# talmolab/Brax-Rodent-Run

Hardware: AMD Instinct MI355X
Metric: env-steps/sec (whole node), rodent 2048 envs/GPU (higher is better)
Workload: dtype f32

## Files before the change

__graft_entry__.py:

```python
import os
import subprocess
import sys

ROOT = os.path.dirname(os.path.abspath(__file__))
PKG = os.path.join(ROOT, "brax-rodent-run_amd")
for p in (ROOT, PKG):
    if p not in sys.path:
        sys.path.insert(0, p)


def build() -> None:
    csrc = os.path.join(PKG, "csrc")
    so = os.path.join(csrc, "librodent_hip.so")
    srcs = [os.path.join(csrc, f) for f in ("rr_api.hip", "rr_kernel.h", "rr_step_body.inc", "rr_mlp.h", "rr_ppo.h", "rr_tanh_normal.h")] + [os.path.join(ROOT, "include", "rodent_rr.h")]
    if not os.path.exists(so) or any(os.path.getmtime(s) > os.path.getmtime(so) for s in srcs):
        cmd = ["hipcc", "--offload-arch=gfx950", "-O2", "-std=c++17", "-shared", "-fPIC", "-fno-slp-vectorize", "-Xclang", "-target-feature",
               "-Xclang", "-load-store-opt", "-o", so, os.path.join(csrc, "rr_api.hip")]
        r = subprocess.run(cmd, stderr=subprocess.PIPE, text=True)
        sys.stderr.write("".join(l for l in r.stderr.splitlines(True) if "not a recognized feature for this target" not in l))
        if r.returncode:
            raise subprocess.CalledProcessError(r.returncode, cmd)
    subprocess.check_call(["make", "-s", "-C", os.path.join(ROOT, "oracle")])
    import rodent_amd
    from rodent_amd import hip
    import ctypes
    lib = ctypes.CDLL(hip.LIB_PATH)
    for sym in hip.EXPORTS:
        getattr(lib, sym)


def smoke() -> None:
    import numpy as np
    import torch
    from rodent_amd import envs, jax_random
    from tests import parity, util
    from tests.oracle_env import OracleRodent

    track = util.synthetic_track()
    N = 64
    env = envs.get_environment("rodent", track_pos=track, num_envs=N, xml_path="rodent_optimized.xml",
                               iterations=8, ls_iterations=8, device="cuda:0")
    keys = jax_random.split(jax_random.PRNGKey(0), N)
    state = env.reset(keys)
    action = parity.f32r(np.random.default_rng(0).uniform(-1, 1, (N, env.action_size)))
    nstate = env.step(state, torch.tensor(action, dtype=torch.float32, device="cuda:0"))
    torch.cuda.synchronize()
    A = OracleRodent("rodent_optimized", N, "f64", (8, 8), track)
    B = OracleRodent("rodent_optimized", N, "f32", (8, 8), track)
    A.reset(keys); B.reset(keys)
    assert np.array_equal(state.pipeline_state.qpos.cpu().numpy(), A.state()["qpos"].astype(np.float32))
    oa, ob = A.step(action), B.step(action)
    assert np.array_equal(nstate.info["cur_frame"].cpu().numpy(), A.cur_frame)
    assert np.array_equal(nstate.done.cpu().numpy(), A.done)
    got = nstate.obs.cpu().numpy().astype(np.float64)
    rows = []
    for k, sl in parity.obs_segments(A.tables).items():
        sc = np.maximum(np.abs(oa[:, sl]).max(1), 1e-3) if k == "cinert" else 1.0
        rows += parity.quantile_rows("obs_" + k, np.abs(got[:, sl] - oa[:, sl]).max(1) / sc, np.abs(ob[:, sl] - oa[:, sl]).max(1) / sc, qs=(0.5,))
    floors = dict(parity.ENV_FLOORS, obs_qpos=parity.ENV_FLOORS["qpos"], obs_qvel=parity.ENV_FLOORS["qvel"])
    parity.check_quantiles(rows, floors)
    assert torch.isfinite(nstate.obs).all()
    print("smoke ok: %d envs, 1 env step (10 substeps); median |qpos - f64 oracle| = %.2e (scalar float32 oracle: %.2e)"
          % (N, rows[0][2], rows[0][3]))


if __name__ == "__main__":
    build()
    if len(sys.argv) > 1 and sys.argv[1] == "smoke":
        smoke()
```

brax-rodent-run_amd/csrc/rr_api.hip:

```cpp
#include "../../include/rodent_rr.h"
#include "rr_kernel.h"
#include "rr_mlp.h"
#include "rr_ppo.h"

#include <atomic>
#include <climits>
#include <cmath>
#include <cstdio>
#include <cstdlib>
#include <cstring>
#include <map>
#include <memory>
#include <mutex>
#include <string>
#include <type_traits>
#include <vector>

static thread_local std::string g_err;
static int fail(int code, const std::string& msg) { g_err = msg; return code; }
extern "C" const char* rr_last_error(void) { return g_err.c_str(); }

#define HIPCHK(x)                                                                                  \
  do {                                                                                             \
    hipError_t e_ = (x);                                                                           \
    if (e_ != hipSuccess) return fail(RR_EHIP, std::string(#x) + ": " + hipGetErrorString(e_));   \
  } while (0)

typedef void (*kern_t)(const RRDims, const RRTables, const RRIO, const int, const int);
struct Entry { int dtype, ndim, dims[4]; size_t count; const void* data; };

struct rr_model {
  std::vector<unsigned char> raw;
  std::map<std::string, Entry> e;
  rr_dims dims;
  RRDims kd;
  std::vector<std::string> dbg_names;
  std::vector<int32_t> dbg_off, dbg_size;
  std::vector<const char*> dbg_cnames;
  int NBS, NVS, NCS;
  bool stage_ok = true;
  int solver = 1;
  bool pair_ok = false;
  RRDims kd_rep;
  bool dyn = false;
  mutable std::atomic<int> live_batches{0};

  const Entry* find(const char* n) const { auto it = e.find(n); return it == e.end() ? nullptr : &it->second; }
  int iscalar(const char* n) const { const Entry* x = find(n); return x ? ((const int32_t*)x->data)[0] : 0; }
  float fscalar(const char* n, int i = 0) const { const Entry* x = find(n); return x ? ((const float*)x->data)[i] : 0.f; }
};

enum Form { F_STEP, F_UNROLL, F_ACTOR, F_EVAL, N_FORMS };
enum Variant { V_PROD, V_DEBUG, V_PROFILE, V_RAND, V_PAIR, V_POSE, N_VARIANTS };
struct Instance { kern_t kern; const char* why = nullptr; bool fixed = false; };

static Instance select(const rr_model* m, Form form, Variant v) {
  const bool s111 = m->NBS == 1 && m->NVS == 1 && m->NCS == 1, s221 = m->NBS == 2 && m->NVS == 2 && m->NCS == 1, s332 = m->NBS == 3 && m->NVS == 3 && m->NCS == 2;
  const bool newton = m->solver == 2, eval = form == F_EVAL, unroll = form != F_STEP, actor = form == F_ACTOR;
  const char *no_diag = "no diagnostic kernel instance for this model", *no_slots = "no kernel instance for this model's slot counts";
  auto no = [](const char* why) { return Instance{nullptr, why}; };
  if (v == V_PAIR && (unroll || newton || !RRDimsRodentNew::matches(m->kd_rep))) return no("no two-wave pair instance for this model / launch form");
  if (v == V_PAIR) return {rr_step_kernel<2, 2, 1, false, false, RRDimsRodentNew, false, false, false, true>, nullptr, true};
  if (unroll && (v == V_DEBUG || v == V_PROFILE)) return no("rr_env_unroll: no diagnostic outputs in a multi-step rollout");
  if (eval) {
    if (newton) return no("rr_env_unroll_eval: the Newton solver has no multi-step instance");
    if (m->pair_ok) return no("rr_env_unroll_eval: two-tree models served by the two-wave pair instance have no multi-step instance");
    if (!s221) return no("rr_env_unroll_eval: only the (2,2,1) slot counts have an evaluation instance");
    if (v == V_RAND) return no("rr_env_unroll_eval: no evaluation instance reads per-env parameters (this batch carries some)");
    if (v == V_POSE) return no("rr_env_unroll_eval: no evaluation instance rewards the pose (this env io carries track_pose); evaluate step by step");
  } else if (v == V_POSE) {
    if (m->dyn) return no("pose tracking: models with candidate-pair contacts (DYN instances) have no pose instance");
    if (m->pair_ok) return no("pose tracking: two-tree models served by the two-wave pair instance have no pose instance");
    if (newton) return no("pose tracking: the Newton solver's instances have no pose instance");
    if (!s221) return no("pose tracking: only the (2,2,1) slot counts have pose instances");
  } else if (v == V_RAND) {
    if (m->dyn) return no("models with candidate-pair contacts (DYN instances) have none");
    if (m->pair_ok) return no("two-tree models served by the two-wave pair instance have none");
    if (newton) return no("the Newton solver's instances have none");
    if (!s221) return no("only the (2,2,1) slot counts have instances with per-env parameters");
  } else if (unroll && (newton || !s221))
    return no("rr_env_unroll: no multi-step kernel instance for this model / solver");
  if (m->dyn) {
    if (v != V_PROD) return no(no_diag);
    if (newton || !s221) return no(no_slots);
    if (eval) return Instance{rr_eval_kernel<RRDims, true>};
    return Instance{actor ? rr_step_kernel<2, 2, 1, false, false, RRDims, false, true, true, false, true>
                    : (unroll ? rr_step_kernel<2, 2, 1, false, false, RRDims, false, true, false, false, true> : rr_step_kernel<2, 2, 1, false, false, RRDims, false, false, false, false, true>)};
  }
  if (v == V_PROFILE && (newton || !s221)) return no(no_diag);
  if (v == V_PROFILE) return RRDimsRodent::matches(m->kd) ? Instance{rr_step_kernel<2, 2, 1, true, false, RRDimsRodent>, nullptr, true} : Instance{rr_step_kernel<2, 2, 1, true, false, RRDims>};
  if (newton)
    return Instance{v == V_DEBUG ? rr_step_kernel<2, 2, 1, false, true, RRDims, true> : rr_step_kernel<2, 2, 1, false, false, RRDims, true>};
  if (v == V_DEBUG)
    return s111 ? Instance{rr_step_kernel<1, 1, 1, false, true, RRDims>} : (s221 ? Instance{rr_step_kernel<2, 2, 1, false, true, RRDims>} : (s332 ? Instance{rr_step_kernel<3, 3, 2, false, true, RRDims>} : no(no_diag)));
  if (!s221) return s111 ? Instance{rr_step_kernel<1, 1, 1, false, false, RRDims>} : (s332 ? Instance{rr_step_kernel<3, 3, 2, false, false, RRDims>} : no(no_slots));
  auto family = [&](auto* t) -> kern_t {
    typedef typename std::remove_pointer<decltype(t)>::type DT;
    if (eval) return rr_eval_kernel<DT>;
    if (v == V_RAND) return actor ? rr_rand_kernel<DT, true, true> : (unroll ? rr_rand_kernel<DT, true> : rr_rand_kernel<DT>);
    if (v == V_POSE) return actor ? rr_pose_kernel<DT, true, true> : (unroll ? rr_pose_kernel<DT, true> : rr_pose_kernel<DT>);
    return actor ? rr_step_kernel<2, 2, 1, false, false, DT, false, true, true> : (unroll ? rr_step_kernel<2, 2, 1, false, false, DT, false, true> : rr_step_kernel<2, 2, 1, false, false, DT>);
  };
  if (RRDimsRodent::matches(m->kd)) return {family((RRDimsRodent*)nullptr), nullptr, true};
  if (RRDimsRodentNew::matches(m->kd)) return {family((RRDimsRodentNew*)nullptr), nullptr, true};
  return Instance{family((RRDims*)nullptr)};
}

static void set_layout(RRDims& k, const RRLayout& L) {
  k.o_qpos = L.o_qpos; k.o_qvel = L.o_qvel; k.o_act = L.o_act; k.o_ctrl = L.o_ctrl; k.o_xpos = L.o_xpos; k.o_xquat = L.o_xquat;
  k.o_cinert = L.o_cinert; k.o_cdof = L.o_cdof; k.o_cvel = L.o_cvel; k.o_qLD = L.o_qLD; k.o_vec = L.o_vec; k.o_x = L.o_x;
  k.o_arm = L.o_arm; k.o_warm = L.o_warm; k.o_qact = L.o_qact; k.o_jlist = L.o_jlist; k.lds_floats = L.lds_floats;
  k.o_H = L.o_H; k.o_Mp = L.o_Mp; k.o_anc = L.o_anc;
}
static bool stage_fits(int nbody, int nv, int con_slots, int nalias) {
  const int pose = std::max(7 * nbody + 4, 6 * nv);
  return 2 * (nalias + 4) <= pose && 2 * (nbody + 8) <= pose && 6 * con_slots <= pose && 4 * con_slots + nv <= std::min(std::min(10 * nbody, 6 * nbody), pose);
}
static bool solve_jobs_fit(const rr_model* m, const char* prefix, int njs, const RRDims& k) {
  return (int)m->find((std::string(prefix) + "k_coljob").c_str())->count == 9 * njs && (int)m->find((std::string(prefix) + "k_rowjob").c_str())->count == 5 * njs &&
         k.lmax <= 16 && k.lmax >= 1 && k.cmax <= 8 && k.rmax <= 8 && k.cmax >= 1;
}

static void layout(rr_model* m) {
  RRDims& k = m->kd;
  const rr_dims& d = m->dims;
  const int con_slots = m->dyn ? m->NCS * RR_LANES : d.ncon;
  const RRLayout L = rr_layout(d.nq, d.nv, d.nu, d.nbody, d.nM, con_slots, m->solver == 2);
  set_layout(k, L);
  k.solver = m->solver;
  k.nfac = m->iscalar(m->solver == 2 ? "k_factor3p_rows" : "k_factor3_rows");
  k.nalias = m->solver == 2 ? 0 : m->iscalar("k_nalias");
  m->dbg_names.clear(); m->dbg_off.clear(); m->dbg_size.clear(); m->dbg_cnames.clear();
  m->stage_ok = stage_fits(d.nbody, d.nv, con_slots, k.nalias);
  if (m->dyn && d.nu > std::max(7 * d.nbody + 4, 6 * d.nv)) m->stage_ok = false;
  int g = 0;
  auto dbg = [&](const char* name, int n) { int r = g; m->dbg_names.push_back(name); m->dbg_off.push_back(g); m->dbg_size.push_back(n); g += n; return r; };
  k.g_xpos = dbg("xpos", 3 * d.nbody); k.g_xquat = dbg("xquat", 4 * d.nbody); k.g_xmat = dbg("xmat", 9 * d.nbody);
  k.g_com = dbg("subtree_com", 6); k.g_cinert = dbg("cinert", 10 * d.nbody); k.g_crb = dbg("crb", 10 * d.nbody);
  k.g_cdof = dbg("cdof", 6 * d.nv); k.g_cvel = dbg("cvel", 6 * d.nbody); k.g_cfrc = dbg("cfrc", 6 * d.nbody);
  k.g_qM = dbg("qM", d.nM); k.g_qLD = dbg("qLD", d.nM); k.g_dinv = dbg("qLDiagInv", d.nv);
  k.g_bias = dbg("qfrc_bias", d.nv); k.g_passive = dbg("qfrc_passive", d.nv); k.g_actuator = dbg("qfrc_actuator", d.nv);
  k.g_smooth = dbg("qfrc_smooth", d.nv); k.g_qacc_smooth = dbg("qacc_smooth", d.nv);
  k.g_con_dist = dbg("con_dist", d.ncon); k.g_con_pos = dbg("con_pos", 3 * d.ncon); k.g_con_frame = dbg("con_frame", 9 * d.ncon);
  k.g_con_D = dbg("con_D", d.ncon); k.g_con_aref = dbg("con_aref", 4 * d.ncon); k.g_lim = dbg("limit_pos_D_aref", 3 * d.nv);
  k.g_qacc = dbg("qacc", d.nv); k.g_qfrc_constraint = dbg("qfrc_constraint", d.nv); k.g_misc = dbg("niter_cost", 2);
  k.g_ls_iters = dbg("ls_iters", 2);
  k.g_solver_end = dbg("solver_end", 2);
  k.g_kaok = dbg("kernarg_ok", 1);
  k.dbg_floats = g;
  for (auto& s : m->dbg_names) m->dbg_cnames.push_back(s.c_str());
  m->dims.lds_bytes = L.lds_floats * (int)sizeof(float);
  m->dims.dbg_floats = g;
  m->dims.solver = m->solver;
  m->dims.fixed_instance = select(m, F_STEP, V_PROD).fixed ? 1 : 0;
}

static void setup_replica(rr_model* m) {
  m->pair_ok = false;
  const char* sw = getenv("RR_PAIR_WAVES");
  if (sw && sw[0] == '0') return;
  static const char* need[] = {"h_dims", "h_k_slots", "h_k_body_i", "h_k_body_f", "h_k_jnt_i", "h_k_jnt_f", "h_k_dof_i", "h_k_dof_f", "h_k_act_f", "h_k_M_ij_k",
                               "h_k_body_anc", "h_k_nround", "h_k_factor3", "h_k_factor3_rows", "h_k_linv", "h_k_linv_rows", "h_k_coljob", "h_k_rowjob", "h_k_jobown",
                               "h_k_solve_lmax", "h_k_solve_cmax", "h_k_solve_rmax", "h_k_nalias", "h_k_con_i", "h_k_con_f", "h_k_con_chain_rows", "h_k_root_mass"};
  for (const char* n : need) if (!m->find(n)) return;
  const int32_t* hd = (const int32_t*)m->find("h_dims")->data;
  const int32_t* sl = (const int32_t*)m->find("h_k_slots")->data;
  if (m->find("h_dims")->count < 8 || sl[0] != 2 || sl[1] != 2 || sl[2] != 1) return;
  if (2 * hd[0] != m->dims.nq || 2 * hd[1] != m->dims.nv || 2 * hd[2] != m->dims.nu || 2 * hd[6] != m->dims.ncon || m->dims.na != m->dims.nu) return;
  RRDims k = m->kd;
  k.nq = hd[0]; k.nv = hd[1]; k.nu = hd[2]; k.nbody = hd[3]; k.njnt = hd[4]; k.nM = hd[5]; k.ncon = hd[6]; k.dmax = hd[7];
  k.nroot = (int)m->find("h_k_root_mass")->count;
  k.nround = m->iscalar("h_k_nround"); k.ninv = m->iscalar("h_k_linv_rows"); k.nfac = m->iscalar("h_k_factor3_rows"); k.nalias = m->iscalar("h_k_nalias");
  k.lmax = m->iscalar("h_k_solve_lmax"); k.cmax = m->iscalar("h_k_solve_cmax"); k.rmax = m->iscalar("h_k_solve_rmax");
  k.obs_dim = k.nq + k.nv + 16 * (k.nbody - 1) + k.nv + 3;
  const RRLayout L = rr_layout(k.nq, k.nv, k.nu, k.nbody, k.nM, k.ncon, false);
  set_layout(k, L);
  k.solver = 1;
  k.nv_scale = m->dims.nv;
  k.lds_bytes_rep = L.lds_floats * 4;
  k.fac_stride = (int)m->find("h_k_factor3")->count; k.inv_stride = (int)m->find("h_k_linv")->count;
  if (!solve_jobs_fit(m, "h_", 2 * RR_LANES, k)) return;
  if (k.nM > RR_LANES * 18 || k.nroot != 1) return;
  if (!stage_fits(k.nbody, k.nv, k.ncon, k.nalias) || 2 * k.lds_bytes_rep + 128 > 64 * 1024) return;
  m->kd_rep = k;
  m->pair_ok = select(m, F_STEP, V_PAIR).kern != nullptr;
}

extern "C" int rr_model_load(const char* path, rr_model** out) {
  if (!path || !out) return fail(RR_EINVAL, "rr_model_load: null argument");
  FILE* f = fopen(path, "rb");
  if (!f) return fail(RR_EIO, std::string("rr_model_load: cannot open ") + path);
  fseek(f, 0, SEEK_END);
  long n = ftell(f);
  fseek(f, 0, SEEK_SET);
  rr_model* m = new rr_model();
  m->raw.resize(n);
  size_t got = fread(m->raw.data(), 1, n, f);
  fclose(f);
  if ((long)got != n || n < 8 || memcmp(m->raw.data(), "RRM1", 4)) { delete m; return fail(RR_EIO, "rr_model_load: not an RRM1 blob"); }
  const unsigned char* raw = m->raw.data();
  uint32_t ne = *(const uint32_t*)(raw + 4);
  if (8 + (size_t)ne * 72 > (size_t)n) { delete m; return fail(RR_EIO, "rr_model_load: truncated header"); }
  const unsigned char* p = raw + 8;
  for (uint32_t i = 0; i < ne; ++i, p += 72) {
    Entry e;
    char name[33] = {0};
    memcpy(name, p, 32);
    e.dtype = *(const uint32_t*)(p + 32);
    e.ndim = *(const uint32_t*)(p + 36);
    for (int k = 0; k < 4; ++k) e.dims[k] = *(const uint32_t*)(p + 40 + 4 * k);
    uint64_t off = *(const uint64_t*)(p + 56), nb = *(const uint64_t*)(p + 64);
    if (off + nb > (uint64_t)n) { delete m; return fail(RR_EIO, "rr_model_load: entry out of range"); }
    e.count = nb / 4;
    e.data = raw + off;
    m->e[name] = e;
  }
  static const char* need[] = {"nq", "nv", "nu", "nbody", "njnt", "ngeom", "nM", "ncon", "nlimit", "nefc", "obs_dim", "k_slots",
                               "k_body_i", "k_body_f", "k_jnt_i", "k_jnt_f", "k_dof_i", "k_dof_f", "k_act_f", "k_M_ij_k", "k_body_anc",
                               "k_nround", "k_factor3", "k_factor3_rows", "k_factor3p", "k_factor3p_rows", "k_nalias", "k_linv", "k_linv_rows", "k_coljob", "k_rowjob",
                               "k_jobown", "k_solve_lmax", "k_solve_cmax", "k_solve_rmax", "k_con_i", "k_con_f", "k_con_chain_packed", "k_con_chain_rows", "k_root_mass",
                               "k_act_i", "k_act_m_i", "k_act_m_f",
                               "dof_depth", "body_depth", "opt_timestep", "opt_gravity", "stat_meaninertia"};
  for (const char* nme : need)
    if (!m->find(nme)) { std::string s = std::string("rr_model_load: blob lacks '") + nme + "'"; delete m; return fail(RR_EIO, s); }
  rr_dims& d = m->dims;
  memset(&d, 0, sizeof(d));
  d.nq = m->iscalar("nq"); d.nv = m->iscalar("nv"); d.nu = m->iscalar("nu"); d.na = m->iscalar("na"); d.nbody = m->iscalar("nbody");
  d.njnt = m->iscalar("njnt"); d.ngeom = m->iscalar("ngeom"); d.nM = m->iscalar("nM"); d.ncon = m->iscalar("ncon");
  d.nlimit = m->iscalar("nlimit"); d.nefc = m->iscalar("nefc"); d.obs_dim = m->iscalar("obs_dim");
  d.iterations = m->iscalar("opt_iterations"); d.ls_iterations = m->iscalar("opt_ls_iterations");
  d.timestep = m->fscalar("opt_timestep");
  const int32_t* sl = (const int32_t*)m->find("k_slots")->data;
  m->NBS = sl[0]; m->NVS = sl[1]; m->NCS = sl[2];
  m->dyn = m->iscalar("k_dyn") != 0;
  if (m->dyn && (m->find("k_con_i")->dims[1] != 8 || m->find("k_con_f")->dims[1] != 32 || (int)m->find("k_con_chain_rows")->count != 10 * (d.ncon + 1) || d.nv >= 128 || d.nu > RR_LANES)) {
    delete m; return fail(RR_EIO, "rr_model_load: candidate-pair tables do not match the DYN kernel instance (stale blob)"); }
  RRDims& k = m->kd;
  memset(&k, 0, sizeof(k));
  k.nq = d.nq; k.nv = d.nv; k.nu = d.nu; k.nbody = d.nbody; k.njnt = d.njnt; k.nM = d.nM; k.ncon = d.ncon;
  int dmax = 0;
  { const Entry* dd = m->find("dof_depth"); for (size_t i = 0; i < dd->count; ++i) dmax = std::max(dmax, ((const int32_t*)dd->data)[i]); }
  k.dmax = dmax;
  k.nroot = (int)m->find("k_root_mass")->count;
  k.nround = m->iscalar("k_nround");
  k.ninv = m->iscalar("k_linv_rows");
  if (d.nM > RR_LANES * (m->NVS == 1 ? 10 : (m->NVS == 2 ? 18 : 35))) { delete m; return fail(RR_EUNSUPPORTED, "rr_model_load: more mass-matrix entries than the kernel's register table"); }
  k.lmax = m->iscalar("k_solve_lmax"); k.cmax = m->iscalar("k_solve_cmax"); k.rmax = m->iscalar("k_solve_rmax");
  if (!solve_jobs_fit(m, "", (m->NVS >= 3 ? m->NVS + 1 : m->NVS) * RR_LANES, k)) {
    delete m; return fail(RR_EIO, "rr_model_load: solve job tables do not match the kernel instance (stale blob)"); }
  k.obs_dim = d.obs_dim; k.iterations = d.iterations; k.ls_iterations = d.ls_iterations;
  k.dt = d.timestep; k.gx = m->fscalar("opt_gravity", 0); k.gy = m->fscalar("opt_gravity", 1); k.gz = m->fscalar("opt_gravity", 2);
  k.tolerance = m->fscalar("opt_tolerance"); k.ls_tolerance = m->fscalar("opt_ls_tolerance");
  k.meaninertia = m->fscalar("stat_meaninertia");
  if (k.nroot > 2) { delete m; return fail(RR_EUNSUPPORTED, "rr_model_load: more than 2 kinematic trees"); }
  if (m->find("k_dof_i")->dims[1] != RR_DOFI) { delete m; return fail(RR_EIO, "rr_model_load: k_dof_i width mismatch (stale blob)"); }
  if (m->find("k_body_i")->dims[1] != RR_BODYI) { delete m; return fail(RR_EIO, "rr_model_load: k_body_i width mismatch (stale blob)"); }
  if (d.nv > 256 || (!m->dyn && d.ncon > 256)) { delete m; return fail(RR_EUNSUPPORTED, "rr_model_load: nv/ncon above the 8-bit table index"); }
  if (m->find("k_con_chain_packed")->dims[1] != m->NCS * RR_LANES) { delete m; return fail(RR_EIO, "rr_model_load: lane-table width mismatch"); }
  k.nv_scale = d.nv > 1 ? d.nv : 1;
  layout(m);
  setup_replica(m);
  *out = m;
  return RR_OK;
}

extern "C" int rr_model_dims(const rr_model* m, rr_dims* out) {
  if (!m || !out) return fail(RR_EINVAL, "rr_model_dims: null argument");
  *out = m->dims;
  return RR_OK;
}
extern "C" int rr_model_set_solver(rr_model* m, int32_t it, int32_t ls) {
  if (!m || it < 0 || ls < 0) return fail(RR_EINVAL, "rr_model_set_solver: bad argument");
  m->dims.iterations = m->kd.iterations = it;
  m->dims.ls_iterations = m->kd.ls_iterations = ls;
  return RR_OK;
}
extern "C" int rr_model_set_solver_type(rr_model* m, int32_t solver) {
  if (!m || (solver != 1 && solver != 2)) return fail(RR_EINVAL, "rr_model_set_solver_type: solver must be 1 (cg) or 2 (newton)");
  if (solver != m->solver && m->live_batches.load() > 0)
    return fail(RR_EINVAL, "rr_model_set_solver_type: batches of this model exist (they hold the LDS layout of the current solver); set the solver before rr_batch_create");
  if (solver == 2 && (!(m->NBS == 2 && m->NVS == 2 && m->NCS == 1) || m->dyn))
    return fail(RR_EUNSUPPORTED, "rr_model_set_solver_type: the Newton instance exists for the single-rodent models only");
  if (solver == 2 && 4 * ((m->dims.nv + 3) & ~3) > std::max(7 * m->dims.nbody + 4, 6 * m->dims.nv))
    return fail(RR_EUNSUPPORTED, "rr_model_set_solver_type: the four Hessian rows do not fit the pose cells");
  m->solver = solver;
  layout(m);
  return RR_OK;
}
extern "C" void rr_model_destroy(rr_model* m) { delete m; }
extern "C" int rr_model_table(const rr_model* m, const char* name, const void** host_ptr, size_t* count, int32_t* dtype) {
  if (!m || !name || !host_ptr) return fail(RR_EINVAL, "rr_model_table: null argument");
  const Entry* e = m->find(name);
  if (!e) return fail(RR_EINVAL, std::string("rr_model_table: the model has no table '") + name + "'");
  *host_ptr = e->data;
  if (count) *count = e->count;
  if (dtype) *dtype = e->dtype;
  return RR_OK;
}
extern "C" int rr_kernarg_layout(int32_t* io_offset, int32_t* io_size, int32_t* total_size) {
  if (io_offset) *io_offset = (int32_t)offsetof(RRKArgs, io);
  if (io_size) *io_size = (int32_t)sizeof(RRIO);
  if (total_size) *total_size = (int32_t)sizeof(RRKArgs);
  return RR_OK;
}

struct rr_batch {
  const rr_model* m;
  int N, device;
  hipStream_t stream;
  RRDims kd;
  RRTables T;
  RRTables T_rep;
  std::vector<void*> dev_allocs;
  bool timing = false;
  std::vector<hipEvent_t> ev0, ev1;
  int npending = 0, ring_head = 0;
  double total_ms = 0;
  int64_t launches = 0;
  unsigned long long* prof = nullptr;
  const int32_t* env_map = nullptr;
  uint32_t* cost = nullptr;
  bool counted = false;
  unsigned* dyn_overflow = nullptr;
  unsigned* bad_states = nullptr;
  unsigned* progress = nullptr;
  float *env_dof_f = nullptr, *env_act_f = nullptr, *env_con_f = nullptr;
  int dbg_flags = 0;
  float* eval_actions = nullptr;
  rr_pose_io pose = {};
  bool has_env_params() const { return env_dof_f || env_act_f || env_con_f; }
};

template <typename Ptr>
static int dev_alloc(rr_batch* b, size_t bytes, Ptr* dst, const void* host = nullptr, size_t host_bytes = 0) {
  void* p = nullptr;
  HIPCHK(hipMalloc(&p, bytes));
  b->dev_allocs.push_back(p);
  if (host_bytes) HIPCHK(hipMemcpy(p, host, host_bytes, hipMemcpyHostToDevice));
  *dst = (Ptr)p;
  return RR_OK;
}
template <typename Ptr>
static int upload(rr_batch* b, const char* name, Ptr* dst) {
  const Entry* e = b->m->find(name);
  return dev_alloc(b, std::max<size_t>(e->count, 1) * 4, dst, e->data, e->count * 4);
}

static int upload_levels(rr_batch* b, const char* name, rr_gi* dst, uint32_t base, uint32_t alias_base, uint32_t nM, int copies = 1, uint32_t rep_bytes = 0) {
  const Entry* e = b->m->find(name);
  std::vector<uint32_t> t((size_t)copies * e->count);
  for (int c = 0; c < copies; ++c) {
    const uint32_t* src = (const uint32_t*)e->data;
    uint32_t* tc = t.data() + (size_t)c * e->count;
    const uint32_t cb = base + (uint32_t)c * rep_bytes, ab = alias_base + (uint32_t)c * rep_bytes;
    for (size_t i = 0; i + 3 < e->count; i += 4) {
      uint32_t f[6] = {src[i] & 0xFFFFu, src[i] >> 16, src[i + 1] & 0xFFFFu, src[i + 1] >> 16, src[i + 2] & 0xFFFFu, src[i + 2] >> 16};
      for (uint32_t& v : f) {
        v = v < nM + 4u ? v * 8u + cb : (v - (nM + 4u)) * 8u + ab;
        if (v > 0xFFFFu) return fail(RR_EUNSUPPORTED, "level schedule does not fit the 16-bit LDS address fields");
      }
      const uint32_t q = src[i + 3];
      if (q > 255u) return fail(RR_EIO, "level schedule: pivot offset out of range (stale blob)");
      tc[i] = f[0] | (f[1] << 16); tc[i + 1] = f[2] | (f[3] << 16); tc[i + 2] = f[4] | (f[5] << 16);
      tc[i + 3] = q * 8u;
    }
  }
  return dev_alloc(b, t.size() * 4, dst, t.data(), t.size() * 4);
}

static int lds_bytes(const rr_model* m, Variant v) { return v == V_PAIR ? 2 * m->kd_rep.lds_bytes_rep + 128 : m->dims.lds_bytes; }

extern "C" int rr_batch_create(const rr_model* m, int32_t num_envs, int32_t device, void* stream, rr_batch** out) {
  if (!m || !out || num_envs <= 0) return fail(RR_EINVAL, "rr_batch_create: bad argument");
  const Instance prod = select(m, F_STEP, V_PROD);
  if (!prod.kern) return fail(RR_EUNSUPPORTED, std::string("rr_batch_create: ") + prod.why);
  HIPCHK(hipSetDevice(device));
  std::unique_ptr<rr_batch, void (*)(rr_batch*)> guard(new rr_batch(), rr_batch_destroy);
  rr_batch* b = guard.get();
  b->m = m; b->N = num_envs; b->device = device; b->stream = (hipStream_t)stream; b->kd = m->kd;
  int rc = 0;
#define UP(T, prefix, field) if ((rc = upload(b, prefix "k_" #field, &T.field))) return rc;
#define UP_REPLICA_TABLES(T, prefix)                                                                                                \
  UP(T, prefix, body_i) UP(T, prefix, jnt_i) UP(T, prefix, dof_i) UP(T, prefix, M_ij_k) UP(T, prefix, body_anc)                     \
  UP(T, prefix, con_chain_rows) UP(T, prefix, coljob) UP(T, prefix, rowjob) UP(T, prefix, jobown) UP(T, prefix, con_i)              \
  UP(T, prefix, body_f) UP(T, prefix, jnt_f) UP(T, prefix, dof_f) UP(T, prefix, act_f) UP(T, prefix, con_f) UP(T, prefix, root_mass)
  UP_REPLICA_TABLES(b->T, "")
  UP(b->T, "", act_i) UP(b->T, "", act_m_i) UP(b->T, "", act_m_f)
  const uint32_t qb = (uint32_t)m->kd.o_qLD * 4u, ab = (uint32_t)m->kd.o_xpos * 4u, nM = (uint32_t)m->dims.nM;
  if ((rc = upload_levels(b, m->solver == 2 ? "k_factor3p" : "k_factor3", &b->T.factor3, qb, ab, nM)) || (rc = upload_levels(b, "k_linv", &b->T.linv, qb, ab, nM))) return rc;
  memset(&b->T_rep, 0, sizeof(b->T_rep));
  if (m->pair_ok) {
    UP_REPLICA_TABLES(b->T_rep, "h_")
    const uint32_t base = (uint32_t)m->kd_rep.o_qLD * 4u, rb = (uint32_t)m->kd_rep.lds_bytes_rep;
    const uint32_t abase = (uint32_t)m->kd_rep.o_xpos * 4u, hnM = (uint32_t)m->kd_rep.nM;
    if ((rc = upload_levels(b, "h_k_factor3", &b->T_rep.factor3, base, abase, hnM, 2, rb)) || (rc = upload_levels(b, "h_k_linv", &b->T_rep.linv, base, abase, hnM, 2, rb))) return rc;
    b->T_rep.anc4 = b->T_rep.M_ij_k;
  }
#undef UP_REPLICA_TABLES
#undef UP
  {
    const Entry *an = m->find("dof_anc"), *ad = m->find("dof_ancadr"), *ma = m->find("dof_Madr");
    std::vector<unsigned char> bytes(((size_t)m->dims.nM + 3) / 4 * 4 + 4, 0);
    if (an && ad && ma) {
      const int32_t *anc = (const int32_t*)an->data, *adr = (const int32_t*)ad->data, *madr = (const int32_t*)ma->data;
      for (int i = 0; i < m->dims.nv; ++i) {
        const int n = adr[i + 1] - adr[i];
        for (int p = 0; p < n; ++p) bytes[madr[i] + p] = (unsigned char)anc[adr[i] + n - 1 - p];
      }
    } else if (m->solver == 2) return fail(RR_EIO, "rr_batch_create: blob lacks the ancestor tables the Newton solver needs");
    if ((rc = dev_alloc(b, bytes.size(), &b->T.anc4, bytes.data(), bytes.size()))) return rc;
  }
  if (!m->stage_ok) return fail(RR_EUNSUPPORTED, "rr_batch_create: 4*ncon + nv exceeds the line-search staging cells (6*nbody)");
  if (m->dims.lds_bytes > 64 * 1024) return fail(RR_EUNSUPPORTED, "rr_batch_create: per-env working set exceeds the 64 KiB of LDS one workgroup may address");
  for (int f = 0; f < N_FORMS; ++f)
    for (int v = 0; v < N_VARIANTS; ++v) {
      const kern_t kk = select(m, (Form)f, (Variant)v).kern;
      if (!kk) continue;
      HIPCHK(hipFuncSetAttribute((const void*)kk, hipFuncAttributeMaxDynamicSharedMemorySize, lds_bytes(m, (Variant)v)));
      hipFuncAttributes fa;
      HIPCHK(hipFuncGetAttributes(&fa, (const void*)kk));
      if (fa.sharedSizeBytes != 0) return fail(RR_EUNSUPPORTED, "rr_batch_create: a step-kernel instance has static LDS (the level schedules need the dynamic segment at address 0)");
    }
  if (m->dyn && (rc = dev_alloc(b, 64, &b->dyn_overflow))) return rc;
  if (m->dyn) HIPCHK(hipMemset(b->dyn_overflow, 0, 64));
  if ((rc = dev_alloc(b, 64, &b->bad_states))) return rc;
  HIPCHK(hipMemset(b->bad_states, 0, 64));
  const char* pace = getenv("RR_PACE");
  if (!(pace && pace[0] == '0') && (rc = dev_alloc(b, 64, &b->progress))) return rc;
  m->live_batches.fetch_add(1);
  b->counted = true;
  *out = guard.release();
  return RR_OK;
}

extern "C" void rr_batch_destroy(rr_batch* b) {
  if (!b) return;
  if (b->counted) b->m->live_batches.fetch_sub(1);
  for (void* p : b->dev_allocs) (void)hipFree(p);
  for (float* p : {b->env_dof_f, b->env_act_f, b->env_con_f, b->eval_actions}) if (p) (void)hipFree(p);
  for (hipEvent_t e : b->ev0) (void)hipEventDestroy(e);
  for (hipEvent_t e : b->ev1) (void)hipEventDestroy(e);
  delete b;
}

#define RR_TIMING_RING 256
static int collect_timing(rr_batch* b, bool all = true) {
  bool first = true;
  while (b->npending > 0) {
    const int i = b->ring_head;
    if (all || (first && hipEventQuery(b->ev1[i]) != hipSuccess)) HIPCHK(hipEventSynchronize(b->ev1[i]));
    else if (hipEventQuery(b->ev1[i]) != hipSuccess) break;
    first = false;
    float ms = 0;
    HIPCHK(hipEventElapsedTime(&ms, b->ev0[i], b->ev1[i]));
    b->total_ms += ms;
    b->launches += 1;
    b->ring_head = (i + 1) % RR_TIMING_RING;
    b->npending -= 1;
  }
  (void)hipGetLastError();
  return RR_OK;
}

struct Launch {
  int mode = 1;
  const rr_state *st = nullptr, *st_in = nullptr;
  const float* ctrl = nullptr;
  int n_frames = 1;
  const rr_env_io* env = nullptr;
  const int32_t* cur_frame_in = nullptr;
  const rr_outputs* out = nullptr;
  const rr_unroll_io* un = nullptr;
  int unroll_T = 0;
  const rr_actor_io* ac = nullptr;
  const rr_eval_io* ev = nullptr;
};
static int check_wrap(const char* who, const rr_unroll_io* w, const char* note = "") {
  if (!w || !w->first.qpos || !w->first.qvel || !w->first.act || !w->first.qacc_warmstart || !w->first_obs || !w->prev_done || !w->steps_in ||
// ... 732 lines not shown
  }
  b->prof = (unsigned long long*)dev_cycles;
  return RR_OK;
}

extern "C" int rr_batch_env_params_supported(const rr_batch* b) {
  if (!b) return fail(RR_EINVAL, "rr_batch_env_params_supported: null batch");
  return select(b->m, F_STEP, V_RAND).kern ? 1 : 0;
}
extern "C" int rr_batch_pose_supported(const rr_batch* b) {
  if (!b) return fail(RR_EINVAL, "rr_batch_pose_supported: null batch");
  const Instance in = select(b->m, F_STEP, V_POSE);
  const char* why = in.kern ? nullptr : in.why;
  if (!why && b->has_env_params()) why = "pose tracking: no pose instance reads per-env parameters (this batch carries some)";
  if (!why && b->prof) why = "pose tracking: no profile build with track_pose";
  if (why) (void)fail(RR_EUNSUPPORTED, std::string("rr_batch_pose_supported: ") + why);
  return why ? 0 : 1;
}
extern "C" int rr_batch_set_pose(rr_batch* b, const rr_pose_io* p) {
  if (!b) return fail(RR_EINVAL, "rr_batch_set_pose: null batch");
  if (!p || (!p->track_pose && !p->pose_metrics)) { b->pose = rr_pose_io{}; return RR_OK; }
  if (!p->track_pose || !p->pose_metrics) return fail(RR_EINVAL, "rr_batch_set_pose: track_pose and pose_metrics go together");
  for (float x : {p->quat_reward_weight, p->quat_reward_scale, p->joint_reward_weight, p->joint_reward_scale})
    if (!(x >= 0.0f) || !std::isfinite(x)) return fail(RR_EINVAL, "rr_batch_set_pose: pose reward weights and scales must be finite and >= 0");
  if (rr_batch_pose_supported(b) != 1) return RR_EUNSUPPORTED;
  b->pose = *p;
  return RR_OK;
}
extern "C" int rr_batch_set_env_params(rr_batch* b, const rr_env_params* p) {
  if (!b) return fail(RR_EINVAL, "rr_batch_set_env_params: null batch");
  const rr_dims& d = b->m->dims;
  const bool any = p && (p->dof_f || p->act_f || p->con_f);
  if (any) {
    const Instance in = select(b->m, F_STEP, V_RAND);
    if (!in.kern) return fail(RR_EUNSUPPORTED, std::string("rr_batch_set_env_params: no kernel instance with per-env parameters: ") + in.why);
    if (b->prof) return fail(RR_EUNSUPPORTED, "rr_batch_set_env_params: no profile build on a batch with per-env parameters (rr_batch_set_profile is on)");
    if (b->pose.track_pose) return fail(RR_EUNSUPPORTED, "rr_batch_set_env_params: pose tracking: no pose instance reads per-env parameters (rr_batch_set_pose is on)");
    if (p->num_envs != b->N) return fail(RR_EINVAL, "rr_batch_set_env_params: num_envs differs from the batch's");
    if ((p->dof_f && p->dof_rows != d.nv) || (p->act_f && p->act_rows != d.nu) || (p->con_f && p->con_rows != d.ncon))
      return fail(RR_EINVAL, "rr_batch_set_env_params: row counts must be the model's nv (dof_f), nu (act_f), ncon (con_f)");
  }
  HIPCHK(hipSetDevice(b->device));
  HIPCHK(hipStreamSynchronize(b->stream));
  float** own[3] = {&b->env_dof_f, &b->env_act_f, &b->env_con_f};
  for (float** o : own) { if (*o) { HIPCHK(hipFree(*o)); *o = nullptr; } }
  if (!any) return RR_OK;
  const float* src[3] = {p->dof_f, p->act_f, p->con_f};
  const size_t bytes[3] = {(size_t)b->N * d.nv * 16 * 4, (size_t)b->N * d.nu * 8 * 4, (size_t)b->N * d.ncon * 26 * 4};
  for (int i = 0; i < 3; ++i) {
    if (!src[i] || !bytes[i]) continue;
    void* q = nullptr;
    HIPCHK(hipMalloc(&q, bytes[i]));
    *own[i] = (float*)q;
    HIPCHK(hipMemcpyAsync(q, src[i], bytes[i], hipMemcpyDeviceToDevice, b->stream));
  }
  HIPCHK(hipStreamSynchronize(b->stream));
  return RR_OK;
}

extern "C" int rr_batch_set_schedule(rr_batch* b, const int32_t* env_map, uint32_t* cost_cycles) {
  if (!b) return fail(RR_EINVAL, "rr_batch_set_schedule: null batch");
  b->env_map = env_map; b->cost = cost_cycles;
  return RR_OK;
}

extern "C" int rr_batch_set_ls_repeat_exit(rr_batch* b, int32_t enable) {
  if (!b) return fail(RR_EINVAL, "rr_batch_set_ls_repeat_exit: null batch");
  b->dbg_flags = enable ? (b->dbg_flags & ~RR_DBG_LS_RUN_REPEATS) : (b->dbg_flags | RR_DBG_LS_RUN_REPEATS);
  return RR_OK;
}

extern "C" int rr_batch_set_solver_trim(rr_batch* b, int32_t enable) {
  if (!b) return fail(RR_EINVAL, "rr_batch_set_solver_trim: null batch");
  b->dbg_flags = enable ? (b->dbg_flags & ~RR_DBG_SOLVER_UNTRIMMED) : (b->dbg_flags | RR_DBG_SOLVER_UNTRIMMED);
  return RR_OK;
}

extern "C" int rr_batch_set_solver_batch(rr_batch* b, int32_t enable) {
  if (!b) return fail(RR_EINVAL, "rr_batch_set_solver_batch: null batch");
  b->dbg_flags = enable ? (b->dbg_flags & ~RR_DBG_SOLVER_UNBATCHED) : (b->dbg_flags | RR_DBG_SOLVER_UNBATCHED);
  return RR_OK;
}

extern "C" int rr_batch_set_timing(rr_batch* b, int32_t enable) {
  if (!b) return fail(RR_EINVAL, "rr_batch_set_timing: null batch");
  HIPCHK(hipSetDevice(b->device));
  if (enable && b->ev0.empty()) {
    for (int i = 0; i < RR_TIMING_RING; ++i) {
      hipEvent_t a, c;
      HIPCHK(hipEventCreate(&a)); b->ev0.push_back(a);
      HIPCHK(hipEventCreate(&c)); b->ev1.push_back(c);
    }
  }
  b->timing = enable != 0;
  b->total_ms = 0; b->launches = 0; b->npending = 0; b->ring_head = 0;
  return RR_OK;
}
extern "C" int rr_batch_kernel_time(rr_batch* b, double* total_ms, int64_t* launches) {
  if (!b) return fail(RR_EINVAL, "rr_batch_kernel_time: null batch");
  int rc = collect_timing(b);
  if (rc) return rc;
  if (total_ms) *total_ms = b->total_ms;
  if (launches) *launches = b->launches;
  return RR_OK;
}
```

brax-rodent-run_amd/csrc/rr_kernel.h:

```cpp
#pragma once
#include <hip/hip_runtime.h>
#include <stdint.h>
#include "rr_tanh_normal.h"

#define RR_LANES 64
#define RR_DOFI 12
#define RR_BODYI 12
#ifndef RR_WIDE
#define RR_WIDE 1
#endif
#ifndef RR_RING
#define RR_RING 6
#endif

#define RR_NPH 24
#ifndef RR_W1
#define RR_W1 2
#define RR_W2 6
#define RR_W3 12
#endif
#ifndef RR_ENV_PRIO
#define RR_ENV_PRIO 1
#endif
#ifndef RR_FACTOR_PRIO
#define RR_FACTOR_PRIO 1
#endif
#ifndef RR_DPP_BLOCK
#define RR_DPP_BLOCK 1
#endif
#ifndef RR_LS_REPEAT_EXIT
#define RR_LS_REPEAT_EXIT 1
#endif
#ifndef RR_JOBS_RESIDENT
#define RR_JOBS_RESIDENT 1
#endif
#ifndef RR_LS_STAGE_ONCE
#define RR_LS_STAGE_ONCE 1
#endif
#define RR_MINVAL 1e-15f
#define RR_MINIMP 0.0001f
#define RR_MAXIMP 0.9999f

struct RRDims {
  int nq, nv, nu, nbody, njnt, nM, ncon, dmax, nroot;
  int obs_dim, iterations, ls_iterations, nfac, nround, ninv, lmax, cmax, rmax;
  float dt, gx, gy, gz, tolerance, ls_tolerance, meaninertia;
  int o_qpos, o_qvel, o_act, o_ctrl, o_xpos, o_xquat, o_cinert, o_cdof, o_cvel,
      o_qLD, o_vec, o_x, o_arm, o_warm, o_qact, o_jlist, lds_floats;
  int o_H, o_Mp, o_anc, solver;
  int nv_scale, fac_stride, inv_stride, lds_bytes_rep;
  int nalias;
  int g_xpos, g_xquat, g_xmat, g_com, g_cinert, g_crb, g_cdof, g_cvel, g_cfrc, g_qM, g_qLD, g_dinv, g_bias, g_passive,
      g_actuator, g_smooth, g_qacc_smooth, g_con_dist, g_con_pos, g_con_frame, g_con_D, g_con_aref, g_lim, g_qacc,
      g_qfrc_constraint, g_misc, g_ls_iters, g_solver_end, g_kaok, dbg_floats;
};

struct RRLayout {
  int o_qpos, o_qvel, o_act, o_ctrl, o_xpos, o_xquat, o_cinert, o_cdof, o_cvel, o_qLD, o_vec, o_x, o_arm, o_warm, o_qact, o_jlist, lds_floats;
  int o_H, o_Mp, o_anc;
};
constexpr int rr_imax(int a, int b) { return a > b ? a : b; }
constexpr int rr_up4(int n) { return (n + 3) & ~3; }
constexpr RRLayout rr_layout(int nq, int nv, int nu, int nbody, int nM, int ncon, bool newton = false) {
  RRLayout k{};
  int o = 0;
  k.o_qpos = o; o += rr_up4(nq);
  k.o_qvel = o; o += rr_up4(nv + 1);
  k.o_act = o; o += rr_up4(nu);
  k.o_ctrl = o; o += rr_up4(nu);
  k.o_xpos = o; o += rr_up4(rr_imax(7 * nbody + 4, 6 * nv));
  k.o_xquat = k.o_xpos + rr_up4(3 * nbody);
  k.o_cinert = o; o += rr_up4(10 * nbody);
  k.o_cdof = o; o += rr_up4(6 * nv + 6);
  k.o_cvel = o; o += rr_up4(6 * nbody);
  k.o_qLD = o; o += rr_up4(rr_imax(rr_imax(2 * (nM + 20), 12 * nbody), 2 * nv));
  k.o_vec = o; o += rr_up4(nv + 16);
  k.o_x = o; o += rr_up4(nv + 16);
  k.o_arm = o; o += rr_up4(2 * nv);
  k.o_warm = o; o += rr_up4(nv);
  k.o_qact = o; o += rr_up4(nv);
  k.o_jlist = o; o += rr_up4(ncon);
  if (newton) {
    k.o_H = o; o += rr_up4(rr_imax(rr_imax(2 * (nM + 20), 12 * nbody), 2 * nv));
    k.o_Mp = o; o += rr_up4(rr_imax(rr_imax(2 * (nM + 20), 12 * nbody), 2 * nv));
    k.o_anc = o; o += rr_up4((nM + 3) / 4 + 1);
  }
  k.lds_floats = o;
  return k;
}

template <int NBODY_, int NCON_, int OBS_>
struct RRDimsFixed : RRDims {
  static constexpr int nq = 74, nv = 73, nu = 30, nbody = NBODY_, njnt = 68, nM = 1119, ncon = NCON_, dmax = 35, nroot = 1, obs_dim = OBS_, nround = 6, lmax = 12, cmax = 6, rmax = 3;
  static constexpr RRLayout LY = rr_layout(nq, nv, nu, nbody, nM, ncon);
  static constexpr int o_qpos = LY.o_qpos, o_qvel = LY.o_qvel, o_act = LY.o_act, o_ctrl = LY.o_ctrl, o_xpos = LY.o_xpos, o_xquat = LY.o_xquat,
                       o_cinert = LY.o_cinert, o_cdof = LY.o_cdof, o_cvel = LY.o_cvel, o_qLD = LY.o_qLD, o_vec = LY.o_vec,
                       o_x = LY.o_x, o_arm = LY.o_arm, o_warm = LY.o_warm, o_qact = LY.o_qact, o_jlist = LY.o_jlist,
                       lds_floats = LY.lds_floats;
  __host__ __device__ RRDimsFixed(const RRDims& d) : RRDims(d) {}
  static bool matches(const RRDims& d) {
    const RRDims& r = d;
    return r.nq == nq && r.nv == nv && r.nu == nu && r.nbody == nbody && r.njnt == njnt && r.nM == nM && r.ncon == ncon && r.dmax == dmax &&
           r.nroot == nroot && r.obs_dim == obs_dim && r.nround == nround && r.lmax == lmax && r.cmax == cmax && r.rmax == rmax && r.o_qpos == o_qpos && r.o_qvel == o_qvel && r.o_act == o_act &&
           r.o_ctrl == o_ctrl && r.o_xpos == o_xpos && r.o_xquat == o_xquat && r.o_cinert == o_cinert && r.o_cdof == o_cdof &&
           r.o_cvel == o_cvel && r.o_qLD == o_qLD && r.o_vec == o_vec && r.o_x == o_x && r.o_arm == o_arm &&
           r.o_warm == o_warm && r.o_qact == o_qact && r.o_jlist == o_jlist && r.lds_floats == lds_floats;
  }
};
typedef RRDimsFixed<66, 59, 1263> RRDimsRodent;
typedef RRDimsFixed<67, 57, 1279> RRDimsRodentNew;

typedef const int __attribute__((address_space(1)))* rr_gi;
typedef const float __attribute__((address_space(1)))* rr_gf;
struct RRTables {
  rr_gi factor3, linv, coljob, rowjob, jobown, body_i, jnt_i, dof_i, M_ij_k, body_anc, con_chain_rows, con_i, anc4;
  rr_gf body_f, jnt_f, dof_f, act_f, con_f, root_mass;
  rr_gi act_i, act_m_i;
  rr_gf act_m_f;
};
struct RRLoopTables { rr_gi factor3, linv, coljob, rowjob, jobown, con_chain_rows; };
static __device__ __forceinline__ RRTables load_tables();
static __device__ __forceinline__ RRDims load_dims();
static __device__ __forceinline__ RRTables load_env_tables(int env, int nv, int nu, int ncon);
typedef const char __attribute__((address_space(1)))* rr_gc;
template <class E>
struct rr_row {
  rr_gc base; unsigned off; int k0;
  __device__ __forceinline__ E operator[](int k) const { return *(const E __attribute__((address_space(1)))*)(base + (size_t)off + (ptrdiff_t)sizeof(E) * (k0 + k)); }
  __device__ __forceinline__ rr_row operator+(int k) const { return rr_row{base, off, k0 + k}; }
};
__device__ __forceinline__ rr_row<int> row_at(rr_gi t, int stride, int idx) { return rr_row<int>{(rr_gc)t, (unsigned)idx * (4u * (unsigned)stride), 0}; }
__device__ __forceinline__ rr_row<float> row_at(rr_gf t, int stride, int idx) { return rr_row<float>{(rr_gc)t, (unsigned)idx * (4u * (unsigned)stride), 0}; }

#define RR_EVAL_RAW 1
#define RR_EVAL_ACTIONS 2
struct RRIO {
  float *qpos, *qvel, *act, *warm;
  const float *qpos_in, *qvel_in, *act_in, *warm_in;
  const int* cur_frame_in;
  const float* ctrl;
  float *o_cinert, *o_cvel, *o_qfrc_actuator, *o_xpos, *o_xmat, *o_com, *dbg;
  float *o_cdist, *o_cpos, *o_cframe;
  const float* track_pos;
  int track_len;
  int* cur_frame;
  float *obs, *reward, *done, *metrics;
  float healthy_reward, ctrl_cost_weight, z_min, z_max;
  int terminate_when_unhealthy;
  unsigned long long* prof;
  const int* env_map;
  unsigned* cost;
  const float *first_qpos, *first_qvel, *first_act, *first_warm, *first_obs;
  const float *prev_done, *steps_in;
  float *steps_out, *trunc_out;
  float episode_length;
  int unroll_T;
  const float *a_obs_in;
  const float *a_mean, *a_std;
  const float *a_W0, *a_b0;
  const float *a_Wt[4], *a_b[4];
  const float *a_Wth, *a_bh;
  const float *a_noise;
  float *a_actions;
  float *t_obs, *t_raw, *t_logp, *t_reward, *t_discount, *t_trunc;
  float a_min_std;
  int a_nh;
  int a_seg, a_pad;
  unsigned* progress;
  unsigned* dyn_overflow;
  unsigned* bad_states;
  float pace_t1, pace_t2, pace_t3;
  int pace_mode;
  const float* env_dof_f;
  const float* env_act_f;
  const float* env_con_f;
  float* e_metrics;
  float* e_qpos_out;
  int mode;
  float bad_state_max;
  int dbg_flags;
  int num_clips;
  const int* clip;
  const float* track_pose;
  float* pose_metrics;
  float pose_quat_w, pose_quat_k, pose_joint_w, pose_joint_k;
};

#define RR_DBG_LS_RUN_REPEATS 1
#define RR_DBG_SOLVER_UNTRIMMED 2
#define RR_DBG_SOLVER_UNBATCHED 4
struct v3 { float x, y, z; };
__device__ __forceinline__ v3 mk3(float x, float y, float z) { v3 r; r.x = x; r.y = y; r.z = z; return r; }
__device__ __forceinline__ v3 ld3(const float* p) { return mk3(p[0], p[1], p[2]); }
__device__ __forceinline__ v3 ld3(const float __attribute__((address_space(1)))* p) { return mk3(p[0], p[1], p[2]); }
__device__ __forceinline__ v3 ld3(const rr_row<float>& p) { return mk3(p[0], p[1], p[2]); }
__device__ __forceinline__ void st3(float* p, v3 a) { p[0] = a.x; p[1] = a.y; p[2] = a.z; }
__device__ __forceinline__ v3 operator+(v3 a, v3 b) { return mk3(a.x + b.x, a.y + b.y, a.z + b.z); }
__device__ __forceinline__ v3 operator-(v3 a, v3 b) { return mk3(a.x - b.x, a.y - b.y, a.z - b.z); }
__device__ __forceinline__ v3 operator*(v3 a, float s) { return mk3(a.x * s, a.y * s, a.z * s); }
__device__ __forceinline__ float dot(v3 a, v3 b) { return a.x * b.x + a.y * b.y + a.z * b.z; }
__device__ __forceinline__ v3 cross(v3 a, v3 b) { return mk3(a.y * b.z - a.z * b.y, a.z * b.x - a.x * b.z, a.x * b.y - a.y * b.x); }

__device__ __forceinline__ void quat_mul(float* r, const float* a, const float* b) {
  float w = a[0] * b[0] - a[1] * b[1] - a[2] * b[2] - a[3] * b[3];
  float x = a[0] * b[1] + a[1] * b[0] + a[2] * b[3] - a[3] * b[2];
  float y = a[0] * b[2] - a[1] * b[3] + a[2] * b[0] + a[3] * b[1];
  float z = a[0] * b[3] + a[1] * b[2] - a[2] * b[1] + a[3] * b[0];
  r[0] = w; r[1] = x; r[2] = y; r[3] = z;
}
__device__ __forceinline__ void quat_to_mat(float* m, const float* q) {
  float w = q[0], x = q[1], y = q[2], z = q[3];
  m[0] = w * w + x * x - y * y - z * z; m[1] = 2 * (x * y - w * z); m[2] = 2 * (x * z + w * y);
  m[3] = 2 * (x * y + w * z); m[4] = w * w - x * x + y * y - z * z; m[5] = 2 * (y * z - w * x);
  m[6] = 2 * (x * z - w * y); m[7] = 2 * (y * z + w * x); m[8] = w * w - x * x - y * y + z * z;
}
__device__ __forceinline__ v3 mat_vec(const float* m, v3 v) {
  return mk3(m[0] * v.x + m[1] * v.y + m[2] * v.z, m[3] * v.x + m[4] * v.y + m[5] * v.z, m[6] * v.x + m[7] * v.y + m[8] * v.z);
}
__device__ __forceinline__ void quat_normalize(float* q) {
  float n = sqrtf(q[0] * q[0] + q[1] * q[1] + q[2] * q[2] + q[3] * q[3]);
  if (n < RR_MINVAL) { q[0] = 1; q[1] = q[2] = q[3] = 0; return; }
  const float inv = 1.0f / n;
  q[0] *= inv; q[1] *= inv; q[2] *= inv; q[3] *= inv;
}
__device__ __forceinline__ void mul_inert_vec(float* res, const float* i, const float* v) {
  res[0] = i[0] * v[0] + i[3] * v[1] + i[4] * v[2] - i[8] * v[4] + i[7] * v[5];
  res[1] = i[3] * v[0] + i[1] * v[1] + i[5] * v[2] + i[8] * v[3] - i[6] * v[5];
  res[2] = i[4] * v[0] + i[5] * v[1] + i[2] * v[2] - i[7] * v[3] + i[6] * v[4];
  res[3] = i[8] * v[1] - i[7] * v[2] + i[9] * v[3];
  res[4] = i[6] * v[2] - i[8] * v[0] + i[9] * v[4];
  res[5] = i[7] * v[0] - i[6] * v[1] + i[9] * v[5];
}
__device__ __forceinline__ void cross_motion(float* res, const float* vel, const float* v) {
  res[0] = -vel[2] * v[1] + vel[1] * v[2];
  res[1] = vel[2] * v[0] - vel[0] * v[2];
  res[2] = -vel[1] * v[0] + vel[0] * v[1];
  res[3] = -vel[2] * v[4] + vel[1] * v[5] - vel[5] * v[1] + vel[4] * v[2];
  res[4] = vel[2] * v[3] - vel[0] * v[5] + vel[5] * v[0] - vel[3] * v[2];
  res[5] = -vel[1] * v[3] + vel[0] * v[4] - vel[4] * v[0] + vel[3] * v[1];
}
__device__ __forceinline__ void cross_force(float* res, const float* vel, const float* f) {
  res[0] = -vel[2] * f[1] + vel[1] * f[2] - vel[5] * f[4] + vel[4] * f[5];
  res[1] = vel[2] * f[0] - vel[0] * f[2] + vel[5] * f[3] - vel[3] * f[5];
  res[2] = -vel[1] * f[0] + vel[0] * f[1] - vel[4] * f[3] + vel[3] * f[4];
  res[3] = -vel[2] * f[4] + vel[1] * f[5];
  res[4] = vel[2] * f[3] - vel[0] * f[5];
  res[5] = -vel[1] * f[3] + vel[0] * f[4];
}
__device__ __forceinline__ float dot6(const float* a, const float* b) {
  float s = a[0] * b[0];
  s += a[1] * b[1]; s += a[2] * b[2]; s += a[3] * b[3]; s += a[4] * b[4]; s += a[5] * b[5];
  return s;
}
__device__ __forceinline__ float dpp_add(float v, const int ctrl_tag) {
  int x = __float_as_int(v), y;
  switch (ctrl_tag) {
    case 0: y = __builtin_amdgcn_update_dpp(0, x, 0xB1, 0xF, 0xF, true); break;
    case 1: y = __builtin_amdgcn_update_dpp(0, x, 0x4E, 0xF, 0xF, true); break;
    case 2: y = __builtin_amdgcn_update_dpp(0, x, 0x141, 0xF, 0xF, true); break;
    case 3: y = __builtin_amdgcn_update_dpp(0, x, 0x140, 0xF, 0xF, true); break;
    case 4: asm("s_nop 1\n\tv_add_f32_dpp %0, %0, %0 row_bcast:15 row_mask:0xa bank_mask:0xf" : "+v"(v)); return v;
    case 5: asm("s_nop 1\n\tv_add_f32_dpp %0, %0, %0 row_bcast:31 row_mask:0xc bank_mask:0xf" : "+v"(v)); return v;
    default: return v;
  }
  return v + __int_as_float(y);
}
__device__ __forceinline__ float wave_sum(float v) {
  v = dpp_add(v, 0); v = dpp_add(v, 1); v = dpp_add(v, 2); v = dpp_add(v, 3); v = dpp_add(v, 4); v = dpp_add(v, 5);
  return __int_as_float(__builtin_amdgcn_readlane(__float_as_int(v), 63));
}
template <int K>
__device__ __forceinline__ void dpp_bcast_stage(float* v) {
  static_assert(K == 3 || K == 4 || K == 6, "instantiated widths");
// ... 628 lines not shown
  static __device__ __forceinline__ void lds_st2(int byte_adr, rr_f2 v) { *(rr_lf2)(size_t)(unsigned)byte_adr = v; }
  struct RowAdr { int a8, p8, b8, d8[4]; };
  template <bool DIV, bool SHIFT>
  static __device__ __forceinline__ RowAdr row_adr(const rr_v4i& e, int delta) {
    const int sh = SHIFT ? delta : 0;
    RowAdr r;
    r.a8 = (e.x & 0xFFFF) + sh; r.b8 = (int)((unsigned)e.x >> 16) + sh;
    r.p8 = DIV ? r.a8 - e.w + 8 : 0;
    r.d8[0] = (e.y & 0xFFFF) + sh; r.d8[1] = (int)((unsigned)e.y >> 16) + sh; r.d8[2] = (e.z & 0xFFFF) + sh; r.d8[3] = (int)((unsigned)e.z >> 16) + sh;
    return r;
  }
  template <bool DIV, bool SHIFT = false>
  __device__ __forceinline__ void run_levels(rr_gi table, int nrows, int delta = 0) {
    typedef const rr_v4i __attribute__((address_space(1)))* rr_gv4;
    typedef const char __attribute__((address_space(1)))* rr_gc;
    const rr_gc tab = (rr_gc)table;
    const unsigned lane16 = 16u * (unsigned)lane;
    constexpr int ROWB = RR_LANES * 16;
    rr_v4i ring[RR_RING];
#pragma unroll
    for (int u = 0; u < RR_RING; ++u) ring[u] = *(rr_gv4)(tab + u * ROWB + lane16);
    RowAdr cur = row_adr<DIV, SHIFT>(ring[0], delta);
    for (int r0 = 0; r0 < nrows; r0 += RR_RING) {
      const rr_gc nxt_rows = tab + (size_t)(r0 + RR_RING) * ROWB;
#pragma unroll
#if RR_WIDE == 2
      for (int u = 0; u < RR_RING; u += 2) {
        if (u && r0 + u >= nrows) break;
        const RowAdr c0 = cur, c1 = row_adr<DIV, SHIFT>(ring[u + 1], delta);
        const rr_f2 va0 = lds_ld2(c0.a8), va1 = lds_ld2(c1.a8);
        rr_f2 vp0 = {1.0f, 1.0f}, vp1 = {1.0f, 1.0f};
        if (DIV) { vp0 = lds_ld2(c0.p8); vp1 = lds_ld2(c1.p8); }
        rr_f2 vb0[4], vo0[4], vb1[4], vo1[4];
#pragma unroll
        for (int j = 0; j < 4; ++j) vb0[j] = lds_ld2(c0.b8 + 8 * j);
#pragma unroll
        for (int j = 0; j < 4; ++j) vo0[j] = lds_ld2(c0.d8[j]);
#pragma unroll
        for (int j = 0; j < 4; ++j) vb1[j] = lds_ld2(c1.b8 + 8 * j);
#pragma unroll
        for (int j = 0; j < 4; ++j) vo1[j] = lds_ld2(c1.d8[j]);
        ring[u] = *(rr_gv4)(nxt_rows + u * ROWB + lane16);
        ring[u + 1] = *(rr_gv4)(nxt_rows + (u + 1) * ROWB + lane16);
        const RowAdr nxt = row_adr<DIV, SHIFT>(ring[(u + 2) % RR_RING], delta);
        rr_f2 t0 = va0, t1 = va1;
        if (DIV) {
          rr_f2 r0_ = {__builtin_amdgcn_rcpf(vp0.x), __builtin_amdgcn_rcpf(vp0.y)}, r1_ = {__builtin_amdgcn_rcpf(vp1.x), __builtin_amdgcn_rcpf(vp1.y)};
          r0_ = r0_ * (2.0f - vp0 * r0_); r1_ = r1_ * (2.0f - vp1 * r1_);
          t0 *= r0_; t1 *= r1_;
        }
#pragma unroll
        for (int j = 0; j < 4; ++j) lds_st2(c0.d8[j], vo0[j] - vb0[j] * t0);
#pragma unroll
        for (int j = 0; j < 4; ++j) lds_st2(c1.d8[j], vo1[j] - vb1[j] * t1);
        cur = nxt;
      }
      if (true) continue;
#endif
      for (int u = 0; u < RR_RING; ++u) {
        if (u && r0 + u >= nrows) break;
        const rr_f2 va = lds_ld2(cur.a8);
        rr_f2 vp = {1.0f, 1.0f};
        if (DIV) vp = lds_ld2(cur.p8);
        rr_f2 vb[4], vo[4];
#pragma unroll
        for (int j = 0; j < 4; ++j) vb[j] = lds_ld2(cur.b8 + 8 * j);
#pragma unroll
        for (int j = 0; j < 4; ++j) vo[j] = lds_ld2(cur.d8[j]);
        ring[u] = *(rr_gv4)(nxt_rows + u * ROWB + lane16);
        const RowAdr nxt = row_adr<DIV, SHIFT>(ring[(u + 1) % RR_RING], delta);
        rr_f2 t = va;
        if (DIV) {
          rr_f2 r = {__builtin_amdgcn_rcpf(vp.x), __builtin_amdgcn_rcpf(vp.y)};
          r = r * (2.0f - vp * r);
          t *= r;
        }
#pragma unroll
        for (int j = 0; j < 4; ++j) lds_st2(cur.d8[j], vo[j] - vb[j] * t);
        cur = nxt;
      }
    }
  }

  __device__ __forceinline__ void factor() {
    int ment[NME];
    load_ment(ment);
    const RRTables T = tables();
    const DT D = phase_dims();
    if (lane < 8) s_qLD[2 * D.nM + lane] = (lane >> 1) == 1 ? 1.0f : ((lane >> 1) == 3 ? -1.0f : 0.0f);
    for (int c = lane; c < 2 * D.nalias; c += RR_LANES) s_buf[c] = 0.0f;
#pragma unroll
    for (int s = 0; s < NVS; ++s) {
      const int d = lane + RR_LANES * s;
      if (d < D.nv) s_qLD[2 * (opaque(dofc1[s]) & 0xFFFF) + 1] += D.dt * row_at(T.dof_f, 16, d)[1];
    }
    sync();
    run_levels<true>(PAIR ? TL.factor3 + rep * D.fac_stride : TL.factor3, D.nfac);
    sync();
#pragma unroll
    for (int s = 0; s < NVS; ++s) {
      const int d = lane + RR_LANES * s;
      const rr_f2 dd = d < D.nv ? *(const rr_f2*)(s_qLD + 2 * (opaque(dofc1[s]) & 0xFFFF)) : rr_f2{1.0f, 1.0f};
      dinv[s] = d < D.nv ? 1.0f / dd.x : 0.0f;
      dinvB[s] = d < D.nv ? 1.0f / dd.y : 0.0f;
      if (d < D.nv) *(rr_f2*)(s_buf + 2 * d) = rr_f2{dinv[s], dinvB[s]};
    }
    sync();
#pragma unroll
    for (int it = 0; it < NME; ++it) {
      const int ij = ment[it];
      if (ij >= 0) {
        const int i = ij & 255, j = ij >> 8;
        if (i != j) *(rr_f2*)(s_qLD + 2 * (lane + RR_LANES * it)) *= *(const rr_f2*)(s_buf + 2 * i);
      }
    }
    sync();
  }

  __device__ __forceinline__ void invert() {
    const DT D = phase_dims();
    run_levels<false>(PAIR ? TL.linv + rep * D.inv_stride : TL.linv, D.ninv);
  }

  static constexpr int NJS = NVS >= 3 ? NVS + 1 : NVS;
  struct Jobs { int cw[NJS][8], ci0[NJS], rb[NJS][4], ra[NJS], own[NVS]; };
  __device__ __forceinline__ void load_jobs(Jobs& j) { load_jobs(j, TL.coljob, TL.rowjob, TL.jobown); }
  template <class P>
  __device__ __forceinline__ void load_jobs(Jobs& j, P coljob, P rowjob, P jobown) {
    constexpr int WJ = NJS * RR_LANES;
    const int ol = opaque(lane);
    const rr_row<int> cj = row_at(coljob, 1, ol), rj = row_at(rowjob, 1, ol), jo = row_at(jobown, 1, ol);
#pragma unroll
    for (int s = 0; s < NJS; ++s) {
#pragma unroll
      for (int k = 0; k < 8; ++k) j.cw[s][k] = 2 * k < D.lmax ? cj[k * WJ + s * RR_LANES] : 0;
      j.ci0[s] = cj[8 * WJ + s * RR_LANES];
#pragma unroll
      for (int k = 0; k < 4; ++k) j.rb[s][k] = 4 * k < D.lmax ? rj[k * WJ + s * RR_LANES] : 0;
      j.ra[s] = rj[4 * WJ + s * RR_LANES];
    }
#pragma unroll
    for (int s = 0; s < NVS; ++s) j.own[s] = ol + RR_LANES * s < D.nv ? jo[RR_LANES * s] : 0;
  }
  static constexpr bool JOBS_RES = RR_JOBS_RESIDENT != 0 && JRES;
  Jobs jobs_res;
  __device__ __forceinline__ void load_jobs_resident() {
    if constexpr (JOBS_RES) { const RRTables T = load_tables(); load_jobs(jobs_res, T.coljob, T.rowjob, T.jobown); }
  }
  __device__ __forceinline__ void jobs_fresh() {
    constexpr bool ALL = rr_same<DT, RRDims>::value;
#pragma unroll
    for (int s = 0; s < NJS; ++s) {
#pragma unroll
      for (int k = 0; k < 8; ++k) if (ALL || 2 * k < D.lmax) asm volatile("" : "+v"(jobs_res.cw[s][k]));
      asm volatile("" : "+v"(jobs_res.ci0[s]));
#pragma unroll
      for (int k = 0; k < 4; ++k) if (ALL || 4 * k < D.lmax) asm volatile("" : "+v"(jobs_res.rb[s][k]));
      asm volatile("" : "+v"(jobs_res.ra[s]));
    }
#pragma unroll
    for (int s = 0; s < NVS; ++s) asm volatile("" : "+v"(jobs_res.own[s]));
  }
  __device__ __forceinline__ float col_piece(const Jobs& j, int s, const float* mat, const float* vec) const {
    const float* v = vec + j.ci0[s];
    float acc = 0.0f;
#pragma unroll
    for (int t = 0; t < 16; ++t)
      if (t < D.lmax) acc += *(const float*)((const char*)mat + ((j.cw[s][t >> 1] >> (16 * (t & 1))) & 0xFFFF)) * v[t];
    return acc;
  }
  __device__ __forceinline__ float row_piece(const Jobs& j, int s, const float* mat, const float* vec) const {
    const float* m_ = (const float*)((const char*)mat + j.ra[s]);
    float acc = 0.0f;
#pragma unroll
    for (int t = 0; t < 16; ++t)
      if (t < D.lmax) acc += m_[2 * t] * vec[(j.rb[s][t >> 2] >> (8 * (t & 3))) & 255];
    return acc;
  }
  static __device__ __forceinline__ float merge_pieces(const float* part, int t0, int c, int cmax) {
    float sum = 0.0f;
// ... 512 lines not shown
      }
    }
#pragma unroll
    for (int s = 0; s < NVS; ++s) {
      float qcs = qc[s];
      if (lim_act[s] && lim_jar[s] < 0) {
        const float f = -lim_D[s] * lim_jar[s];
        part[0] += lim_D[s] * lim_jar[s] * lim_jar[s];
        qcs += lim_sign[s] * f;
      }
      qfrc_con[s] = qcs;
      part[1] += (Ma[s] - qfrc_smooth[s]) * (qacc[s] - qacc_smooth[s]);
    }
    solver_sum_n<2>(part);
    gauss = 0.5f * part[1];
    prev_cost = cost;
    cost = 0.5f * part[0] + gauss;
  }

  __device__ __forceinline__ void newton_hessian() {
    const int RS = (D.nv + 3) & ~3;
    for (int e = lane; e < D.nM + 20; e += RR_LANES) *(rr_f2*)(s_H + 2 * e) = *(const rr_f2*)(s_Mp + 2 * e);
    float cd[NVS][6];
#pragma unroll
    for (int s = 0; s < NVS; ++s) {
      const int d = lane + RR_LANES * s;
#pragma unroll
      for (int k = 0; k < 6; ++k) cd[s][k] = d < D.nv ? s_cdof[6 * d + k] : 0.0f;
    }
    sync();
#pragma unroll
    for (int s = 0; s < NVS; ++s) {
      if (lim_act[s] && lim_jar[s] < 0) { rr_f2* h = (rr_f2*)(s_H + 2 * (opaque(dofc1[s]) & 0xFFFF)); *h += rr_f2{lim_D[s], lim_D[s]}; }
    }
#pragma unroll
    for (int cs = 0; cs < NCS; ++cs) {
      unsigned long long mask = __ballot(con_act[cs]);
      while (mask) {
        const int l = __builtin_ctzll(mask);
        mask &= mask - 1;
        auto bc = [&](float v) { return __int_as_float(__builtin_amdgcn_readlane(__float_as_int(v), l)); };
        const float mu = bc(con_mu[cs]), Dc = bc(con_D[cs]);
        const v3 off = mk3(bc(con_off[cs][0]), bc(con_off[cs][1]), bc(con_off[cs][2]));
        const v3 fn = mk3(bc(con_fr[cs][0]), bc(con_fr[cs][1]), bc(con_fr[cs][2])), f1 = mk3(bc(con_fr[cs][3]), bc(con_fr[cs][4]), bc(con_fr[cs][5])),
                 f2 = mk3(bc(con_fr[cs][6]), bc(con_fr[cs][7]), bc(con_fr[cs][8]));
        float a[4];
#pragma unroll
        for (int k = 0; k < 4; ++k) a[k] = bc(con_jar[cs][k]) < 0 ? Dc : 0.0f;
        const int ld = __builtin_amdgcn_readlane(con_leaf[cs], l);
        float r[NVS][4];
        bool on[NVS];
#pragma unroll
        for (int s = 0; s < NVS; ++s) {
          const int d = lane + RR_LANES * s;
          on[s] = d < D.nv && d <= ld && ld <= (opaque(dofc1[s]) >> 16);
          const v3 jp = mk3(cd[s][3], cd[s][4], cd[s][5]) + cross(mk3(cd[s][0], cd[s][1], cd[s][2]), off);
          const float jn = dot(fn, jp), j1 = dot(f1, jp), j2 = dot(f2, jp);
          r[s][0] = on[s] ? jn + mu * j1 : 0.0f; r[s][1] = on[s] ? jn - mu * j1 : 0.0f;
          r[s][2] = on[s] ? jn + mu * j2 : 0.0f; r[s][3] = on[s] ? jn - mu * j2 : 0.0f;
          if (d < D.nv) {
#pragma unroll
            for (int k = 0; k < 4; ++k) s_buf[k * RS + d] = r[s][k];
          }
        }
        sync();
#pragma unroll
        for (int s = 0; s < NVS; ++s) {
          if (s > 0 && ld < RR_LANES * s) continue;
          if (on[s]) {
            const int madr = opaque(dofc1[s]) & 0xFFFF, dep = opaque(dofc0[s]) & 255;
            const float w0 = a[0] * r[s][0], w1 = a[1] * r[s][1], w2 = a[2] * r[s][2], w3 = a[3] * r[s][3];
            for (int p = 0; p <= dep; ++p) {
              const int j = s_anc[madr + p];
              const float v = w0 * s_buf[j] + w1 * s_buf[RS + j] + w2 * s_buf[2 * RS + j] + w3 * s_buf[3 * RS + j];
              rr_f2* h = (rr_f2*)(s_H + 2 * (madr + p));
              *h += rr_f2{v, v};
            }
          }
        }
        sync();
      }
    }
  }
  __device__ __forceinline__ void newton_factor() {
    const int delta = (int)((D.o_H - D.o_qLD) * sizeof(float));
    int ment[NME];
    load_ment(ment);
    if (lane < 8) s_H[2 * D.nM + lane] = (lane >> 1) == 1 ? 1.0f : 0.0f;
    sync();
    run_levels<true, true>(TL.factor3, D.nfac, delta);
    sync();
#pragma unroll
    for (int s = 0; s < NVS; ++s) {
      const int d = lane + RR_LANES * s;
      dinvH[s] = d < D.nv ? 1.0f / s_H[2 * (opaque(dofc1[s]) & 0xFFFF)] : 0.0f;
      if (d < D.nv) *(rr_f2*)(s_buf + 2 * d) = rr_f2{dinvH[s], dinvH[s]};
    }
    sync();
#pragma unroll
    for (int it = 0; it < NME; ++it) {
      const int ij = ment[it];
      if (ij >= 0) {
        const int i = ij & 255, j = ij >> 8;
        if (i != j) *(rr_f2*)(s_H + 2 * (lane + RR_LANES * it)) *= *(const rr_f2*)(s_buf + 2 * i);
      }
    }
    sync();
    run_levels<false, true>(TL.linv, D.ninv, delta);
    sync();
  }

  __device__ __forceinline__ void form_gradient() {
#pragma unroll
    for (int s = 0; s < NVS; ++s) grad[s] = Ma[s] - qfrc_smooth[s] - qfrc_con[s];
  }
  __device__ __forceinline__ void solve_gradient() {
#pragma unroll
    for (int s = 0; s < NVS; ++s) Mgrad[s] = grad[s];
    for (int rep = 0; rep < RR_REP_SOLVE; ++rep) { float t_[NVS]; for (int s = 0; s < NVS; ++s) t_[s] = grad[s]; ldl_solve(t_); }
    if (NEWTON) {
      newton_hessian();
      newton_factor();
      ldl_solve_on(Mgrad, s_H, dinvH);
    } else {
      ldl_solve(Mgrad);
    }
  }

  __device__ __forceinline__ void direction(int niter, const float* pm, float gg) {
    if (niter == 0) {
#pragma unroll
      for (int s = 0; s < NVS; ++s) { search[s] = -Mgrad[s]; mv[s] = -grad[s]; }
    } else {
      float bt[2] = {0.0f, gg};
#pragma unroll
      for (int s = 0; s < NVS; ++s) bt[0] += grad[s] * (Mgrad[s] - pm[s]);
      solver_sum_n<2>(bt);
      const float beta = NEWTON ? 0.0f : fmaxf(0.0f, bt[0] / fmaxf(RR_MINVAL, bt[1]));
#pragma unroll
      for (int s = 0; s < NVS; ++s) { search[s] = -Mgrad[s] + beta * search[s]; mv[s] = -grad[s] + beta * mv[s]; }
    }
  }

  __device__ __forceinline__ void ctx_create(bool at_smooth, bool rows_kept, bool walk) {
    if (!rows_kept) {
      put_vec(qacc);
      jac_mul(con_jar, s_vec);
#pragma unroll
      for (int cs = 0; cs < NCS; ++cs)
#pragma unroll
        for (int k = 0; k < 4; ++k) con_jar[cs][k] -= con_aref[cs][k];
#pragma unroll
      for (int s = 0; s < NVS; ++s) lim_jar[s] = lim_sign[s] * qacc[s] - lim_aref[s];
    }
    if (at_smooth) {
#pragma unroll
      for (int s = 0; s < NVS; ++s) Ma[s] = qfrc_smooth[s];
    } else {
#pragma unroll
      for (int s = 0; s < NVS; ++s) Ma[s] = Ma_warm[s];
    }
    cost = INFINITY; prev_cost = 0.0f;
    update_constraint(walk);
  }

  static constexpr int KR = 4 * NCS + NVS;
  template <int NP, bool COST>
  __device__ __forceinline__ void ls_eval(const float* alpha, const float* qg, LSPoint* out, int R, const float* rjr, const float* rjv,
                                          const float* rD) {
    constexpr int NQ = COST ? 3 : 2;
    float q[NQ * NP];
#pragma unroll
    for (int i = 0; i < NQ * NP; ++i) q[i] = 0.0f;
#pragma unroll
    for (int r = 0; r < KR; ++r) {
      if (r * RR_LANES < R) {
        const float jr = rjr[r], jv = rjv[r], Dv = rD[r];
        const float q0 = 0.5f * jr * jr * Dv, q1 = jv * jr * Dv, q2 = 0.5f * jv * jv * Dv;
#pragma unroll
        for (int i = 0; i < NP; ++i)
          if (jr + alpha[i] * jv < 0) { q[NQ * i] += q1; q[NQ * i + 1] += q2; if (COST) q[NQ * i + 2] += q0; }
      }
    }
    solver_sum_n<NQ * NP>(q);
#pragma unroll
    for (int i = 0; i < NP; ++i) {
      const float q1 = qg[1] + q[NQ * i], q2 = qg[2] + q[NQ * i + 1];
      const float a = alpha[i];
      out[i].alpha = a;
      out[i].cost = COST ? a * a * q2 + a * q1 + (qg[0] + q[NQ * i + (COST ? 2 : 0)]) : 0.0f;
      out[i].d0 = 2.0f * a * q2 + q1;
      out[i].d1 = 2.0f * q2 + (q2 == 0.0f ? RR_MINVAL : 0.0f);
    }
  }

  int ls_R = 0;
  int ls_cpos[NCS], ls_lpos[NVS];
  float ls_rD[KR];
  __device__ __forceinline__ void ls_stage() {
    int R = 0;
#pragma unroll
    for (int cs = 0; cs < NCS; ++cs) {
      const unsigned long long m = __ballot(con_act[cs]);
      const int pos = R + 4 * (int)__builtin_amdgcn_mbcnt_hi((unsigned)(m >> 32), __builtin_amdgcn_mbcnt_lo((unsigned)m, 0u));
      R += 4 * __popcll(m);
// ... 143 lines not shown
        if constexpr (PROF || DBG) ls_left = so_ls_iterations - 1 - it;
        it = so_ls_iterations;
        break;
      }
#endif
    }
#if RR_LS_REPEAT_EXIT
    work += 3 * (1 + (R > RR_LANES ? 1 : 0)) * (it < so_ls_iterations ? it + 1 : it);
#endif
    if constexpr (PROF) { pt[20] += (unsigned)ls_ran; pt[21] += (unsigned)ls_left; }
    if constexpr (DBG) { dbg_ls_ran += ls_ran; dbg_ls_left += ls_left; }
    {
      const float a2[2] = {lo.alpha, hi.alpha};
      LSPoint f2[2];
      ls_eval<2, true>(a2, qg, f2, R, rjr, rjv, rD);
      lo.cost = f2[0].cost; hi.cost = f2[1].cost;
    }
    stamp<PROF>(19);
    const bool improved = uni((lo.cost < p0.cost) || (hi.cost < p0.cost));
    const float alpha = lo.cost < hi.cost ? lo.alpha : hi.alpha;
    if (improved) {
#pragma unroll
      for (int s = 0; s < NVS; ++s) { qacc[s] += search[s] * alpha; Ma[s] += mv[s] * alpha; lim_jar[s] += lim_jv[s] * alpha; }
#pragma unroll
      for (int cs = 0; cs < NCS; ++cs)
#pragma unroll
        for (int k = 0; k < 4; ++k) con_jar[cs][k] += con_jv[cs][k] * alpha;
    }
  }

  template <bool PROF, bool DBG = false>
  __device__ __forceinline__ int solve() {
    {
      const DT Dl = phase_dims();
      so_tolerance = Dl.tolerance; so_ls_tolerance = Dl.ls_tolerance; so_meaninertia = Dl.meaninertia;
      so_iterations = Dl.iterations; so_ls_iterations = Dl.ls_iterations; so_nv_scale = Dl.nv_scale;
    }
    const float scale = 1.0f / (so_meaninertia * (float)so_nv_scale);
    const bool untrimmed = DBG && (dbg_flags & RR_DBG_SOLVER_UNTRIMMED) != 0;
    const bool unbatched = DBG && (dbg_flags & RR_DBG_SOLVER_UNBATCHED) != 0;
    if (RR_LS_STAGE_ONCE && !unbatched) ls_stage();
    float cost_smooth = 0.0f;
    bool use_smooth = false;
    float jar0[NCS][4], ljar0[NVS];
#pragma unroll
    for (int cs = 0; cs < NCS; ++cs)
#pragma unroll
      for (int k = 0; k < 4; ++k) jar0[cs][k] = 0.0f;
#pragma unroll
    for (int s = 0; s < NVS; ++s) ljar0[s] = 0.0f;
#pragma nounroll
    for (int ph = 0; ph < 3; ++ph) {
      if (ph == 2 && !use_smooth) break;
#pragma unroll
      for (int s = 0; s < NVS; ++s) qacc[s] = ph != 1 ? qacc_smooth[s] : (lane + RR_LANES * s < D.nv ? s_warm[lane + RR_LANES * s] : 0.0f);
      const bool rows_kept = ph == 2 && !untrimmed;
      if (rows_kept) {
#pragma unroll
        for (int cs = 0; cs < NCS; ++cs)
#pragma unroll
          for (int k = 0; k < 4; ++k) con_jar[cs][k] = jar0[cs][k];
#pragma unroll
        for (int s = 0; s < NVS; ++s) lim_jar[s] = ljar0[s];
      }
      ctx_create(ph != 1, rows_kept, ph != 0 || untrimmed);
      if (ph == 0) {
        cost_smooth = cost;
#pragma unroll
        for (int cs = 0; cs < NCS; ++cs)
#pragma unroll
          for (int k = 0; k < 4; ++k) jar0[cs][k] = con_jar[cs][k];
#pragma unroll
        for (int s = 0; s < NVS; ++s) ljar0[s] = lim_jar[s];
      }
      if (ph == 1) use_smooth = uni(!(cost < cost_smooth));
    }
    if constexpr (DBG) dbg_solver_end = use_smooth ? 1 : 0;
    form_gradient();
    int niter = 0;
    float pm[NVS], gg = 0.0f;
#pragma unroll
    for (int s = 0; s < NVS; ++s) pm[s] = 0.0f;
    while (true) {
      if (untrimmed) { solve_gradient(); direction(niter, pm, gg); }
      const float improvement = (prev_cost - cost) * scale;
      float g2 = 0.0f;
#pragma unroll
      for (int s = 0; s < NVS; ++s) g2 += grad[s] * grad[s];
      const float gradient = sqrtf(solver_sum(g2)) * scale;
      bool done = niter >= so_iterations;
      done |= improvement < so_tolerance;
      done |= gradient < so_tolerance;
      if (uni(done)) {
        if constexpr (DBG) dbg_solver_end |= (niter >= so_iterations ? 2 : 0) | (uni(improvement < so_tolerance) ? 4 : 0) | (uni(gradient < so_tolerance) ? 8 : 0);
        break;
      }
      if constexpr (PROF) { if (niter) stamp<PROF>(12); }
      if (!untrimmed) {
        solve_gradient();
        if constexpr (PROF) { if (niter) stamp<PROF>(11); }
        direction(niter, pm, gg);
      }
      if constexpr (PROF) { if (niter) stamp<PROF>(12); else stamp<PROF>(8); }
      for (int rep = 0; rep < RR_REP_LS; ++rep) linesearch<false>();
      linesearch<PROF, DBG>();
      stamp<PROF>(9);
      gg = 0.0f;
#pragma unroll
      for (int s = 0; s < NVS; ++s) { gg += grad[s] * Mgrad[s]; pm[s] = Mgrad[s]; }
      for (int rep = 0; rep < RR_REP_UC; ++rep) { const float pc = prev_cost, c0 = cost; update_constraint(); prev_cost = pc; cost = c0; }
      update_constraint();
      stamp<PROF>(10);
      form_gradient();
      ++niter;
    }
#pragma unroll
    for (int s = 0; s < NVS; ++s) { const int d = lane + RR_LANES * s; if (d < D.nv) s_warm[d] = qacc[s]; }
    return niter;
  }

  __device__ __forceinline__ void euler() {
    float qa[NVS];
#pragma unroll
    for (int s = 0; s < NVS; ++s) qa[s] = qfrc_smooth[s] + qfrc_con[s];
    ldl_solve<true>(qa);
    const RRTables T = tables();
    const DT D = phase_dims();
#pragma unroll
    for (int s = 0; s < NVS; ++s) {
      const int d = lane + RR_LANES * s;
      if (d < D.nv) {
        const int u = DYN ? -1 : row_at(T.dof_i, RR_DOFI, d)[7];
        if (u >= 0) {
          auto af = row_at(T.act_f, 8, u);
          const float c = fminf(fmaxf(s_ctrl[u], af[5]), af[6]);
          s_act[u] += D.dt * ((c - s_act[u]) / fmaxf(af[4], RR_MINVAL));
        }
        s_qvel[d] += D.dt * qa[s];
      }
    }
    if (DYN && lane < D.nu) {
      auto af = row_at(T.act_f, 8, lane);
      const float c = fminf(fmaxf(s_ctrl[lane], af[5]), af[6]);
      s_act[lane] += D.dt * ((c - s_act[lane]) / fmaxf(af[4], RR_MINVAL));
    }
    sync();
#pragma unroll
    for (int s = 0; s < NVS; ++s) {
      const int d = lane + RR_LANES * s;
      if (d < D.nv) {
        const int kind = row_at(T.dof_i, RR_DOFI, d)[2], qadr = row_at(T.dof_i, RR_DOFI, d)[6];
        if (kind == 6 || kind < 3) {
          s_qpos[qadr] += D.dt * s_qvel[d];
        } else if (kind == 3) {
          const v3 w = ld3(s_qvel + d);
          const float n = sqrtf(dot(w, w));
          v3 ax = mk3(0, 0, 0);
          if (n > RR_MINVAL) ax = w * (1.0f / n);
          const float ang = D.dt * n;
          float sn, cs;
          sincosf(ang * 0.5f, &sn, &cs);
          float qr[4] = {cs, ax.x * sn, ax.y * sn, ax.z * sn}, q0[4], qn[4];
          for (int k = 0; k < 4; ++k) q0[k] = s_qpos[qadr + k];
          quat_mul(qn, q0, qr);
          quat_normalize(qn);
          for (int k = 0; k < 4; ++k) s_qpos[qadr + k] = qn[k];
        }
      }
    }
    sync();
  }
};

struct RRKArgs { RRDims D; RRTables T; RRIO io; int num_envs, n_frames; };
constexpr size_t rr_align_up(size_t x, size_t a) { return (x + a - 1) / a * a; }
static_assert(alignof(RRDims) == 4 && alignof(RRTables) == 8 && alignof(RRIO) == 8, "argument alignments the kernarg layout relies on");
static_assert(offsetof(RRKArgs, T) == rr_align_up(sizeof(RRDims), alignof(RRTables)), "RRTables follows RRDims at its natural alignment");
static_assert(offsetof(RRKArgs, io) == rr_align_up(offsetof(RRKArgs, T) + sizeof(RRTables), alignof(RRIO)), "RRIO follows RRTables at its natural alignment");
static_assert(offsetof(RRKArgs, num_envs) == offsetof(RRKArgs, io) + sizeof(RRIO) && sizeof(RRIO) % 8 == 0, "scalars follow RRIO without padding");
static_assert(offsetof(RRIO, clip) % 8 == 0 && offsetof(RRIO, clip) + sizeof(const int*) == offsetof(RRIO, track_pose), "the pose members follow the clip ids without padding");
static_assert(offsetof(RRIO, pose_joint_k) + sizeof(float) == sizeof(RRIO), "the pose members close RRIO without padding");
static __device__ __forceinline__ RRTables load_tables() {
// ... 166 lines not shown
```

brax-rodent-run_amd/csrc/rr_step_body.inc:

```
  static_assert(!PAIR || (!PROF && !DBG && !NEWTON && !UNROLL && !ACTOR), "PAIR: production physics instance only");
  static_assert(!DYN || (!PROF && !DBG && !NEWTON && !PAIR), "DYN: production instances only (single-step, multi-step, multi-step with the actor)");
  static_assert(!ACTOR || UNROLL, "the actor lives in the multi-step instances");
  static_assert(!POSE || (!RAND && !EVAL && !PROF && !DBG && !NEWTON && !PAIR && !DYN), "POSE: production CG instances of the floor-contact models only");
  static_assert(!EVAL || (ACTOR && !RAND && !PROF && !DBG && !NEWTON && !PAIR), "EVAL: a form of the production multi-step instance with the actor");
  extern __shared__ __attribute__((aligned(16))) float lds[];
  int env = blockIdx.x;
  if (env >= num_envs) return;
  const DT D(Dk);
  const int wrep = PAIR ? __builtin_amdgcn_readfirstlane((int)(threadIdx.x >> 6)) : 0;
  Wave<NBS, NVS, NCS, DT, NEWTON, PAIR, DYN, RAND, !DBG> w(D, Tk, PAIR ? lds + wrep * (D.lds_bytes_rep >> 2) : lds);
  int lane = threadIdx.x & (RR_LANES - 1);
  if (PAIR) { w.rep = wrep; w.s_xc = lds + 2 * (D.lds_bytes_rep >> 2); }
  RRIO io = load_io();
  if (io.env_map) {
    env = __builtin_amdgcn_readfirstlane(io.env_map[env]);
    if ((unsigned)env >= (unsigned)num_envs) return;
  }
  if (RAND) w.renv = env;
  if (DBG) {
    const RRIO ref_io = io_kernarg;
    bool same = true;
    for (unsigned i = 0; i < sizeof(RRIO) / sizeof(int); ++i) same &= ((const int*)&io)[i] == ((const int*)&ref_io)[i];
    if (ref_io.dbg && lane == 0) ref_io.dbg[(size_t)env * D.dbg_floats + D.g_kaok] = same ? 1.0f : 0.0f;
    if (!same) return;
// ... 92 lines not shown
    }
    for (int rep = 0; rep < RR_REP_KIN; ++rep) w.kinematics();
    w.kinematics();
    w.template stamp<PROF>(0);
    w.com_pos();
    w.template stamp<PROF>(1);
    if (last) {
#pragma unroll
      for (int k = 0; k < 4; ++k) xq1[k] = w.s_xquat[4 + k];
      if (io.o_xpos) for (int e = lane; e < 3 * D.nbody; e += RR_LANES) io.o_xpos[(size_t)env * 3 * D.nbody + e] = w.s_xpos[e];
      if (io.o_xmat || dg) {
        for (int b = lane; b < D.nbody; b += RR_LANES) {
          float q[4], mm[9];
          for (int k = 0; k < 4; ++k) q[k] = w.s_xquat[4 * b + k];
          quat_to_mat(mm, q);
          for (int k = 0; k < 9; ++k) {
            if (io.o_xmat) io.o_xmat[(size_t)env * 9 * D.nbody + 9 * b + k] = mm[k];
            if (dg) dg[D.g_xmat + 9 * b + k] = mm[k];
          }
        }
      }
      if (io.o_com && lane == 0) for (int k = 0; k < 3; ++k) io.o_com[(size_t)env * 3 + k] = w.com0[k];
      if (dg) {
        for (int e = lane; e < 3 * D.nbody; e += RR_LANES) dg[D.g_xpos + e] = w.s_xpos[e];
        for (int e = lane; e < 4 * D.nbody; e += RR_LANES) dg[D.g_xquat + e] = w.s_xquat[e];
        for (int e = lane; e < 10 * D.nbody; e += RR_LANES) dg[D.g_cinert + e] = w.s_cinert[e];
        for (int e = lane; e < 6 * D.nv; e += RR_LANES) dg[D.g_cdof + e] = w.s_cdof[e];
        if (lane == 0) { for (int k = 0; k < 3; ++k) { dg[D.g_com + k] = w.com0[k]; dg[D.g_com + 3 + k] = w.com1[k]; } }
      }
    }
    {
      float *od = nullptr, *op = nullptr, *of = nullptr;
      if (DBG && last) {
        od = io.o_cdist ? io.o_cdist + (size_t)env * D.ncon : nullptr;
        op = io.o_cpos ? io.o_cpos + (size_t)env * 3 * D.ncon : nullptr;
        of = io.o_cframe ? io.o_cframe + (size_t)env * 9 * D.ncon : nullptr;
      }
      if (DYN) w.contact_geometry_dyn();
      else w.contact_geometry(dg, od, op, of);
    }
    w.velocity_sweep();
    w.template stamp<PROF>(2);
    if (last) {
      if (io.o_cinert) for (int e = lane; e < 10 * D.nbody; e += RR_LANES) io.o_cinert[(size_t)env * 10 * D.nbody + e] = w.s_cinert[e];
      if (io.o_cvel) for (int e = lane; e < 6 * D.nbody; e += RR_LANES) io.o_cvel[(size_t)env * 6 * D.nbody + e] = w.s_cvel[e];
      if (io.obs) {
        float* ob = (EVAL ? io.t_obs + ((size_t)env * 2 + ((ut + 1) & 1)) * D.obs_dim : ACTOR ? io.t_obs + rr_traj_obs(io, num_envs, env, rr_traj(io, ut).u, rr_traj(io, ut).t + 1) * D.obs_dim : io.obs + (size_t)env * D.obs_dim) + D.nq + D.nv;
        for (int i = lane; i < 10 * (D.nbody - 1); i += RR_LANES) ob[i] = w.s_cinert[10 + i];
        ob += 10 * (D.nbody - 1);
        for (int i = lane; i < 6 * (D.nbody - 1); i += RR_LANES) ob[i] = w.s_cvel[6 + i];
      }
      if (dg) for (int e = lane; e < 6 * D.nbody; e += RR_LANES) dg[D.g_cvel + e] = w.s_cvel[e];
    }
    w.backward_sweep();
    w.template stamp<PROF>(3);
    w.smooth_forces(bias, passive);
    if (dg) {
      for (int e = lane; e < 10 * D.nbody; e += RR_LANES) dg[D.g_crb + e] = w.s_crb[e];
      for (int e = lane; e < 6 * D.nbody; e += RR_LANES) dg[D.g_cfrc + e] = e < 6 ? 0.0f : w.s_cfrc[e];
    }
    w.contact_jobs();
    w.env_prio();
    w.sync();
    for (int rep = 0; rep < RR_REP_MM; ++rep) w.mass_matrix();
    w.mass_matrix();
    w.template stamp<PROF>(4);
    if (dg) for (int e = lane; e < D.nM; e += RR_LANES) dg[D.g_qM + e] = w.s_qLD[2 * e];
    if (NEWTON) {
      for (int e = lane; e < D.nM + 20; e += RR_LANES) *(rr_f2*)(w.s_Mp + 2 * e) = *(const rr_f2*)(w.s_qLD + 2 * e);
      w.sync();
    }
    {
      float wv[NVS];
#pragma unroll
      for (int s = 0; s < NVS; ++s) { const int d = lane + RR_LANES * s; wv[s] = d < D.nv ? w.s_warm[d] : 0.0f; }
      w.put_vec(wv);
      w.load_jobs_resident();
      w.mul_m(w.Ma_warm);
    }
#if RR_FACTOR_PRIO
    if ((w.lag_mode & 8) && w.lag_prio == 0) __builtin_amdgcn_s_setprio(2);
    else __builtin_amdgcn_s_setprio(3);
#endif
    w.factor();
    if (dg) for (int e = lane; e < D.nM; e += RR_LANES) dg[D.g_qLD + e] = w.s_qLD[2 * e];
    w.invert();
    w.env_prio();
    w.template stamp<PROF>(5);
#pragma unroll
    for (int s = 0; s < NVS; ++s) w.qacc_smooth[s] = w.qfrc_smooth[s];
    w.ldl_solve(w.qacc_smooth);
    w.template stamp<PROF>(6);
    if (dg) {
#pragma unroll
      for (int s = 0; s < NVS; ++s) {
        const int d = lane + RR_LANES * s;
        if (d < D.nv) {
          dg[D.g_dinv + d] = w.dinv[s]; dg[D.g_bias + d] = bias[s]; dg[D.g_passive + d] = passive[s];
          dg[D.g_actuator + d] = w.s_qact[d]; dg[D.g_smooth + d] = w.qfrc_smooth[s];
          dg[D.g_qacc_smooth + d] = w.qacc_smooth[s];
        }
      }
    }
    w.constraint_rows(dg);
    w.template stamp<PROF>(7);
    if (DBG) { w.dbg_flags = io.dbg_flags; w.dbg_ls_ran = w.dbg_ls_left = 0; }
    niter = w.template solve<PROF, DBG>();
    w.template stamp<PROF>(12);
    if (dg) {
#pragma unroll
      for (int s = 0; s < NVS; ++s) {
        const int d = lane + RR_LANES * s;
        if (d < D.nv) { dg[D.g_qacc + d] = w.qacc[s]; dg[D.g_qfrc_constraint + d] = w.qfrc_con[s]; }
      }
      if (lane == 0) {
        dg[D.g_misc] = (float)niter; dg[D.g_misc + 1] = w.cost;
        dg[D.g_ls_iters] = (float)w.dbg_ls_ran; dg[D.g_ls_iters + 1] = (float)w.dbg_ls_left;
        dg[D.g_solver_end] = (float)(w.dbg_solver_end & 1); dg[D.g_solver_end + 1] = (float)(w.dbg_solver_end >> 1);
      }
    }
    if (mode & 1) w.euler();
    w.template stamp<PROF>(13);
    if (UNROLL && !last) {
      const RRIO iop = load_io();
      if (iop.progress && (iop.pace_mode & 4)) {
        unsigned seen = 0;
        if (lane == 0) seen = __hip_atomic_fetch_add(iop.progress, 1u, __ATOMIC_RELAXED, __HIP_MEMORY_SCOPE_AGENT) + 1u;
        seen = (unsigned)__builtin_amdgcn_readfirstlane((int)seen);
        const float behind = ((float)seen / (float)num_envs - (float)(ut * frames + f + 1)) / (float)frames;
        w.lag_prio = behind > iop.pace_t3 ? 3 : (behind > iop.pace_t2 ? 2 : (behind > iop.pace_t1 ? 1 : 0));
        w.lag_mode = iop.pace_mode;
      }
    }
  }

  w.template stamp<PROF>(14);
  lane = opaque(lane); w.lane = lane;
  asm volatile("" : "+s"(env));
  if (RAND) w.renv = env;
  if (!PAIR) {
    const float bad_max = load_io_member<float>(offsetof(RRIO, bad_state_max));
    mode &= 3;
    if (bad_max > 0.0f && !(mode & 2)) {
      bool b = false;
      for (int i = lane; i < D.nq; i += RR_LANES) b |= !(fabsf(w.s_qpos[i]) <= bad_max);
      for (int i = lane; i < D.nv; i += RR_LANES) b |= !(fabsf(w.s_qvel[i]) <= bad_max);
      if (__builtin_amdgcn_ballot_w64(b) != 0) {
        mode |= 4;
        if (lane == 0) __hip_atomic_fetch_add(load_io_member<unsigned*>(offsetof(RRIO, bad_states)), 1u, __ATOMIC_RELAXED, __HIP_MEMORY_SCOPE_AGENT);
      }
    }
  }
  io = load_io();
  if (PROF && io.prof && lane == 0) for (int i = 0; i < RR_NPH; ++i) io.prof[(size_t)env * RR_NPH + i] = w.pt[i];
  if (UNROLL) u_work += (unsigned)w.work;
  if (UNROLL && DYN) u_overflow |= w.dyn_overflow;
  if (io.cost && lane == 0 && wrep == 0) io.cost[env] = (UNROLL ? u_work : (unsigned)w.work) | (DYN && (UNROLL ? u_overflow : w.dyn_overflow) ? 0x80000000u : 0u);
  if (DYN && w.dyn_overflow && io.dyn_overflow && lane == 0) __hip_atomic_fetch_add(io.dyn_overflow, 1u, __ATOMIC_RELAXED, __HIP_MEMORY_SCOPE_AGENT);
  if (!UNROLL) {
    for (int i = lane; i < D.nq; i += RR_LANES) io.qpos[(size_t)senv * D.nq + i] = w.s_qpos[i];
    for (int i = lane; i < D.nv; i += RR_LANES) io.qvel[(size_t)senv * D.nv + i] = w.s_qvel[i];
    for (int i = lane; i < D.nu; i += RR_LANES) io.act[(size_t)senv * D.nu + i] = w.s_act[i];
#pragma unroll
    for (int s = 0; s < NVS; ++s) {
      const int d = lane + RR_LANES * s;
      if (d < D.nv) {
        io.warm[(size_t)senv * D.nv + d] = w.s_warm[d];
// ... 161 lines not shown
```

brax-rodent-run_amd/rodent_amd/hip.py:

```python
from __future__ import annotations

import ctypes as C
import os
from typing import Dict, Optional

import torch

_HERE = os.path.dirname(os.path.abspath(__file__))
LIB_PATH = os.environ.get("RR_LIB") or os.path.join(os.path.dirname(_HERE), "csrc", "librodent_hip.so")


class RRDims(C.Structure):
    _fields_ = [(n, C.c_int32) for n in ("nq", "nv", "nu", "na", "nbody", "njnt", "ngeom", "nM", "ncon", "nlimit",
                                         "nefc", "obs_dim", "iterations", "ls_iterations", "lds_bytes", "dbg_floats")] \
        + [("timestep", C.c_float), ("solver", C.c_int32), ("fixed_instance", C.c_int32)]


class RRState(C.Structure):
    _fields_ = [(n, C.c_void_p) for n in ("qpos", "qvel", "act", "qacc_warmstart")]


class RROutputs(C.Structure):
    _fields_ = [(n, C.c_void_p) for n in ("cinert", "cvel", "qfrc_actuator", "xpos", "xmat", "subtree_com", "debug",
                                                "contact_dist", "contact_pos", "contact_frame")]


class RRMlpNet(C.Structure):
    _fields_ = [("weights", C.POINTER(C.c_void_p)), ("biases", C.POINTER(C.c_void_p)), ("sizes", C.POINTER(C.c_int32)), ("nlayers", C.c_int32)]


class RREnvIO(C.Structure):
    _fields_ = [("track_pos", C.c_void_p), ("track_len", C.c_int32), ("cur_frame", C.c_void_p), ("obs", C.c_void_p),
                ("reward", C.c_void_p), ("done", C.c_void_p), ("metrics", C.c_void_p), ("healthy_reward", C.c_float),
                ("ctrl_cost_weight", C.c_float), ("healthy_z_min", C.c_float), ("healthy_z_max", C.c_float),
                ("terminate_when_unhealthy", C.c_int32), ("bad_state_max", C.c_float)]


class RREnvIOClips(C.Structure):
    _fields_ = RREnvIO._fields_ + [("clip", C.c_void_p), ("num_clips", C.c_int32)]


class RRPoseIO(C.Structure):
    _fields_ = [("track_pose", C.c_void_p), ("pose_metrics", C.c_void_p), ("quat_reward_weight", C.c_float), ("quat_reward_scale", C.c_float),
                ("joint_reward_weight", C.c_float), ("joint_reward_scale", C.c_float)]


class RRUnrollIO(C.Structure):
    _fields_ = [("first", RRState), ("first_obs", C.c_void_p), ("prev_done", C.c_void_p), ("steps_in", C.c_void_p), ("steps_out", C.c_void_p),
                ("truncation_out", C.c_void_p), ("episode_length", C.c_float)]


class RRActorIO(C.Structure):
    _fields_ = [(n, C.c_void_p) for n in ("obs_in", "mean", "std", "w0", "b0")] + [("hidden_wt", C.c_void_p * 4), ("hidden_b", C.c_void_p * 4)] + \
        [(n, C.c_void_p) for n in ("head_wt", "head_b", "noise", "actions_out", "traj_obs", "traj_raw_action", "traj_log_prob", "traj_reward",
                                   "traj_discount", "traj_truncation")] + [("min_std", C.c_float), ("nhidden", C.c_int32), ("segment_length", C.c_int32)]


class RREvalIO(C.Structure):
    _fields_ = [("eval_metrics", C.c_void_p), ("obs_ring", C.c_void_p), ("qpos_out", C.c_void_p), ("raw_env", C.c_int32)]


class RREnvParams(C.Structure):
    _fields_ = [("dof_f", C.c_void_p), ("act_f", C.c_void_p), ("con_f", C.c_void_p), ("dof_rows", C.c_int32), ("act_rows", C.c_int32),
                ("con_rows", C.c_int32), ("num_envs", C.c_int32)]


class RRDwItem(C.Structure):
    _fields_ = [(n, C.c_void_p) for n in ("delta", "act", "act_rows", "mean", "std", "delta_colsum")] + \
        [("M", C.c_int32), ("O", C.c_int32), ("I", C.c_int32), ("grad", C.c_void_p)]


class RRPpoCfg(C.Structure):
    _fields_ = [(n, C.c_float) for n in ("entropy_cost", "discounting", "reward_scaling", "gae_lambda", "clipping_epsilon", "min_std")] + \
        [("normalize_advantage", C.c_int32)]


EXPORTS = ["rr_model_load", "rr_model_dims", "rr_model_set_solver", "rr_model_set_solver_type", "rr_model_destroy", "rr_model_table", "rr_kernarg_layout", "rr_batch_create",
           "rr_batch_destroy", "rr_pipeline_init", "rr_pipeline_step", "rr_env_step", "rr_env_reset", "rr_pipeline_step_to", "rr_env_step_to", "rr_batch_contact_overflow", "rr_batch_bad_states", "rr_batch_unroll_supported", "rr_env_unroll", "rr_env_unroll_policy", "rr_batch_eval_supported", "rr_env_unroll_eval", "rr_batch_pose_supported", "rr_batch_set_pose",
           "rr_compute_gae", "rr_mlp_forward", "rr_ppo_loss_workspace_bytes", "rr_ppo_loss", "rr_policy_act_workspace_bytes", "rr_policy_act", "rr_policy_sample", "rr_policy_backward_workspace_bytes", "rr_policy_backward", "rr_mlp_silu_backward_workspace_bytes", "rr_mlp_silu_backward", "rr_mlp_value_backward_workspace_bytes", "rr_mlp_policy_backward", "rr_mlp_policy_backward_workspace_bytes", "rr_mlp_value_backward", "rr_mlp_weight_grad_workspace_bytes", "rr_mlp_weight_grad", "rr_mlp_weight_grad_batch_workspace_bytes", "rr_mlp_weight_grad_batch", "rr_obs_moments_workspace_bytes", "rr_obs_moments", "rr_wrap_episode_autoreset", "rr_debug_layout", "rr_batch_set_schedule", "rr_batch_set_env_params", "rr_batch_env_params_supported", "rr_batch_set_profile", "rr_batch_set_ls_repeat_exit", "rr_batch_set_solver_trim", "rr_batch_set_solver_batch", "rr_batch_set_timing", "rr_batch_kernel_time", "rr_last_error"]

_lib = None


def lib():
    global _lib
    if _lib is None:
        if not os.path.exists(LIB_PATH):
            raise RuntimeError(f"{LIB_PATH} not found: run `python -c 'import __graft_entry__ as g; g.build()'`")
        L = C.CDLL(LIB_PATH)
        L.rr_last_error.restype = C.c_char_p
        L.rr_model_load.argtypes = [C.c_char_p, C.POINTER(C.c_void_p)]
        L.rr_model_dims.argtypes = [C.c_void_p, C.POINTER(RRDims)]
        L.rr_model_set_solver.argtypes = [C.c_void_p, C.c_int32, C.c_int32]
        L.rr_model_set_solver_type.argtypes = [C.c_void_p, C.c_int32]
        L.rr_model_destroy.argtypes = [C.c_void_p]
        L.rr_model_destroy.restype = None
        L.rr_model_table.argtypes = [C.c_void_p, C.c_char_p, C.POINTER(C.c_void_p), C.POINTER(C.c_size_t), C.POINTER(C.c_int32)]
        L.rr_kernarg_layout.argtypes = [C.POINTER(C.c_int32)] * 3
        L.rr_batch_create.argtypes = [C.c_void_p, C.c_int32, C.c_int32, C.c_void_p, C.POINTER(C.c_void_p)]
        L.rr_batch_destroy.argtypes = [C.c_void_p]
        L.rr_batch_destroy.restype = None
        L.rr_pipeline_init.argtypes = [C.c_void_p, C.POINTER(RRState), C.POINTER(RROutputs)]
        L.rr_pipeline_step.argtypes = [C.c_void_p, C.POINTER(RRState), C.c_void_p, C.c_int32, C.POINTER(RROutputs)]
        L.rr_env_step.argtypes = [C.c_void_p, C.POINTER(RRState), C.c_void_p, C.c_int32, C.POINTER(RREnvIOClips),
                                  C.POINTER(RROutputs)]
        L.rr_pipeline_step_to.argtypes = [C.c_void_p, C.POINTER(RRState), C.POINTER(RRState), C.c_void_p, C.c_int32, C.POINTER(RROutputs)]
        L.rr_env_step_to.argtypes = [C.c_void_p, C.POINTER(RRState), C.POINTER(RRState), C.c_void_p, C.c_int32, C.POINTER(RREnvIOClips),
                                     C.c_void_p, C.POINTER(RROutputs)]
        L.rr_batch_unroll_supported.argtypes = [C.c_void_p, C.c_int32]
        L.rr_batch_contact_overflow.argtypes = [C.c_void_p, C.POINTER(C.c_int64)]
        L.rr_batch_bad_states.argtypes = [C.c_void_p, C.POINTER(C.c_int64)]
        L.rr_env_unroll.argtypes = [C.c_void_p, C.POINTER(RRState), C.POINTER(RRState), C.c_void_p, C.c_int32, C.c_int32, C.POINTER(RREnvIOClips),
                                    C.c_void_p, C.POINTER(RRUnrollIO)]
        L.rr_env_unroll_policy.argtypes = [C.c_void_p, C.POINTER(RRState), C.POINTER(RRState), C.c_int32, C.c_int32, C.POINTER(RREnvIOClips), C.c_void_p,
                                           C.POINTER(RRUnrollIO), C.POINTER(RRActorIO)]
        L.rr_batch_eval_supported.argtypes = [C.c_void_p]
        L.rr_env_unroll_eval.argtypes = [C.c_void_p, C.POINTER(RRState), C.POINTER(RRState), C.c_int32, C.c_int32, C.POINTER(RREnvIOClips), C.c_void_p,
                                         C.POINTER(RRUnrollIO), C.POINTER(RRActorIO), C.POINTER(RREvalIO)]
        L.rr_env_reset.argtypes = [C.c_void_p, C.POINTER(RRState), C.POINTER(RREnvIOClips), C.POINTER(RROutputs)]
        L.rr_debug_layout.argtypes = [C.c_void_p, C.POINTER(C.POINTER(C.c_char_p)), C.POINTER(C.POINTER(C.c_int32)),
                                      C.POINTER(C.POINTER(C.c_int32))]
        L.rr_compute_gae.argtypes = [C.c_void_p] * 5 + [C.c_int32, C.c_int32, C.c_float, C.c_float, C.c_void_p, C.c_void_p, C.c_void_p]
        L.rr_mlp_forward.argtypes = [C.c_void_p, C.c_void_p, C.c_int32, C.c_int32, C.c_void_p, C.c_void_p, C.POINTER(RRMlpNet), C.POINTER(RRMlpNet),
                                     C.c_void_p, C.c_void_p, C.c_void_p, C.c_void_p, C.c_void_p]
        L.rr_ppo_loss_workspace_bytes.argtypes = [C.c_int32, C.c_int32]
        L.rr_ppo_loss_workspace_bytes.restype = C.c_size_t
        L.rr_ppo_loss.argtypes = [C.c_void_p] * 9 + [C.c_int32] * 3 + [C.POINTER(RRPpoCfg)] + [C.c_void_p] * 4 + [C.c_size_t, C.c_void_p]
        L.rr_policy_act_workspace_bytes.argtypes = [C.c_int32]
        L.rr_policy_act_workspace_bytes.restype = C.c_size_t
        L.rr_policy_act.argtypes = [C.c_void_p, C.c_void_p, C.c_int32, C.c_int32, C.c_void_p, C.c_void_p, C.POINTER(RRMlpNet), C.c_void_p, C.c_float,
                                    C.c_void_p, C.c_void_p, C.c_void_p, C.c_void_p, C.c_void_p, C.c_size_t, C.c_void_p]
        L.rr_policy_sample.argtypes = [C.c_void_p, C.c_void_p, C.c_int32, C.c_int32, C.c_float, C.c_void_p, C.c_void_p, C.c_void_p, C.c_void_p]
        L.rr_policy_backward_workspace_bytes.argtypes = [C.c_int32, C.c_int32]
        L.rr_policy_backward_workspace_bytes.restype = C.c_size_t
        L.rr_policy_backward.argtypes = [C.c_void_p, C.c_void_p, C.POINTER(C.c_void_p), C.c_int32, C.c_int32, C.c_int32, C.c_void_p, C.c_int32, C.c_void_p,
                                         C.POINTER(C.c_void_p), C.c_void_p, C.c_size_t, C.c_void_p]
        L.rr_mlp_silu_backward_workspace_bytes.argtypes = [C.c_int32, C.c_int32]
        L.rr_mlp_silu_backward_workspace_bytes.restype = C.c_size_t
        L.rr_mlp_silu_backward.argtypes = [C.c_void_p, C.c_void_p, C.c_int32, C.c_int32, C.c_void_p, C.c_void_p, C.c_void_p, C.c_void_p, C.c_size_t, C.c_void_p]
        L.rr_mlp_value_backward_workspace_bytes.argtypes = [C.c_int32, C.c_int32]
        L.rr_mlp_value_backward_workspace_bytes.restype = C.c_size_t
        L.rr_mlp_value_backward.argtypes = [C.c_void_p, C.c_void_p, C.POINTER(C.c_void_p), C.c_int32, C.c_int32, C.c_void_p, C.c_void_p,
                                            C.POINTER(C.c_void_p), C.c_void_p, C.c_size_t, C.c_void_p]
        L.rr_mlp_policy_backward_workspace_bytes.argtypes = [C.c_int32, C.c_int32]
        L.rr_mlp_policy_backward_workspace_bytes.restype = C.c_size_t
        L.rr_mlp_policy_backward.argtypes = [C.c_void_p, C.c_void_p, C.POINTER(C.c_void_p), C.c_int32, C.c_int32, C.c_int32, C.c_int32, C.c_void_p, C.c_void_p,
                                             C.POINTER(C.c_void_p), C.c_void_p, C.c_size_t, C.c_void_p]
        L.rr_mlp_weight_grad_workspace_bytes.argtypes = [C.c_int32] * 3
        L.rr_mlp_weight_grad_workspace_bytes.restype = C.c_size_t
        L.rr_mlp_weight_grad.argtypes = [C.c_void_p] * 6 + [C.c_int32] * 3 + [C.c_void_p, C.c_void_p, C.c_size_t, C.c_void_p]
        L.rr_mlp_weight_grad_batch_workspace_bytes.argtypes = [C.POINTER(RRDwItem), C.c_int32]
        L.rr_mlp_weight_grad_batch_workspace_bytes.restype = C.c_size_t
        L.rr_mlp_weight_grad_batch.argtypes = [C.POINTER(RRDwItem), C.c_int32, C.c_void_p, C.c_size_t, C.c_void_p]
        L.rr_wrap_episode_autoreset.argtypes = [C.c_int32, C.c_int32, C.POINTER(C.c_void_p), C.POINTER(C.c_void_p), C.POINTER(C.c_int32)] + \
            [C.c_void_p] * 5 + [C.c_float, C.c_float, C.c_void_p]
        L.rr_obs_moments_workspace_bytes.argtypes = [C.c_int64, C.c_int32, C.c_int32]
        L.rr_obs_moments_workspace_bytes.restype = C.c_size_t
        L.rr_obs_moments.argtypes = [C.c_void_p, C.c_int64, C.c_int32, C.c_int32, C.c_int32, C.c_void_p, C.c_void_p, C.c_void_p, C.c_size_t, C.c_void_p]
        L.rr_batch_set_profile.argtypes = [C.c_void_p, C.c_void_p]
        L.rr_batch_set_schedule.argtypes = [C.c_void_p, C.c_void_p, C.c_void_p]
        L.rr_batch_set_env_params.argtypes = [C.c_void_p, C.POINTER(RREnvParams)]
        L.rr_batch_env_params_supported.argtypes = [C.c_void_p]
        L.rr_batch_pose_supported.argtypes = [C.c_void_p]
        L.rr_batch_set_pose.argtypes = [C.c_void_p, C.POINTER(RRPoseIO)]
        L.rr_batch_set_ls_repeat_exit.argtypes = [C.c_void_p, C.c_int32]
        L.rr_batch_set_solver_trim.argtypes = [C.c_void_p, C.c_int32]
        L.rr_batch_set_solver_batch.argtypes = [C.c_void_p, C.c_int32]
        L.rr_batch_set_timing.argtypes = [C.c_void_p, C.c_int32]
        L.rr_batch_kernel_time.argtypes = [C.c_void_p, C.POINTER(C.c_double), C.POINTER(C.c_int64)]
        _lib = L
    return _lib


def _check(rc):
    if rc < 0:
        raise RuntimeError(f"librodent_hip: {lib().rr_last_error().decode()} (status {rc})")
    return rc


def _ptr(t: Optional[torch.Tensor], dtype=torch.float32, numel: Optional[int] = None):
    if t is None:
        return None
    if not t.is_cuda or t.dtype != dtype or not t.is_contiguous():
        raise ValueError(f"expected a contiguous {dtype} device tensor, got {t.dtype} on {t.device}")
    if numel is not None and t.numel() != numel:
        raise ValueError(f"tensor has {t.numel()} elements, expected {numel}")
    return t.data_ptr()


def _dp(t: Optional[torch.Tensor]):
    return t.data_ptr() if t is not None else None


def head_columns(P: int) -> int:
    return 64 if P <= 64 else 128


_scratch: dict = {}


def _ws(bufs: Optional[dict], call: str, dev, shape_key, nbytes: int, dtype=torch.float32, shape=None) -> torch.Tensor:
    store = _scratch if bufs is None else bufs
    key = (call, dev, torch.cuda.current_stream(dev).cuda_stream, shape_key)
    if key not in store:
        item = dtype.itemsize
        store[key] = torch.empty(shape if shape is not None else ((nbytes + item - 1) // item,), dtype=dtype, device=dev)
    return store[key]


class Model:

    def __init__(self, blob_path: str, iterations: Optional[int] = None, ls_iterations: Optional[int] = None, solver: Optional[str] = None):
        self.h = C.c_void_p()
        _check(lib().rr_model_load(blob_path.encode(), C.byref(self.h)))
        if solver is not None:
            _check(lib().rr_model_set_solver_type(self.h, {"cg": 1, "newton": 2}[solver.lower()]))
        if iterations is not None:
            d = self.dims
            _check(lib().rr_model_set_solver(self.h, iterations, ls_iterations if ls_iterations is not None else d.ls_iterations))

    def table(self, name: str):
        import numpy as np
        ptr, cnt, dt = C.c_void_p(), C.c_size_t(), C.c_int32()
        _check(lib().rr_model_table(self.h, name.encode(), C.byref(ptr), C.byref(cnt), C.byref(dt)))
        ctype = C.c_float if dt.value == 0 else C.c_int32
        return np.ctypeslib.as_array(C.cast(ptr, C.POINTER(ctype)), shape=(cnt.value,)).copy()

    @property
    def dims(self) -> RRDims:
        d = RRDims()
        _check(lib().rr_model_dims(self.h, C.byref(d)))
        return d

    def __del__(self):
        try:
            if self.h:
                lib().rr_model_destroy(self.h)
        except Exception:
            pass


class Batch:

    def __init__(self, model: Model, num_envs: int, device: Optional[torch.device] = None):
        if not torch.cuda.is_available():
            raise RuntimeError("rodent_amd.hip.Batch needs a GPU (no CPU fallback)")
        self.model = model
        self.device = torch.device("cuda", torch.cuda.current_device()) if device is None else torch.device(device)
        self.N = int(num_envs)
        self.dims = model.dims
        self.h = C.c_void_p()
        self._pose = None
        with torch.cuda.device(self.device):
            stream = torch.cuda.current_stream().cuda_stream
        _check(lib().rr_batch_create(model.h, self.N, self.device.index or 0, C.c_void_p(stream), C.byref(self.h)))

    def __del__(self):
        try:
            if self.h:
                lib().rr_batch_destroy(self.h)
        except Exception:
            pass

    def zeros_state(self) -> Dict[str, torch.Tensor]:
        d, N, dev = self.dims, self.N, self.device
        return dict(qpos=torch.zeros(N, d.nq, device=dev), qvel=torch.zeros(N, d.nv, device=dev),
                    act=torch.zeros(N, d.na, device=dev), qacc_warmstart=torch.zeros(N, d.nv, device=dev))

    def _state(self, st) -> RRState:
        d, N = self.dims, self.N
        return RRState(_ptr(st["qpos"], numel=N * d.nq), _ptr(st["qvel"], numel=N * d.nv),
                       _ptr(st["act"], numel=N * d.na), _ptr(st["qacc_warmstart"], numel=N * d.nv))

    def _outputs(self, out) -> Optional[RROutputs]:
        if not out:
            return None
        d, N = self.dims, self.N
        sizes = dict(cinert=10 * d.nbody, cvel=6 * d.nbody, qfrc_actuator=d.nv, xpos=3 * d.nbody, xmat=9 * d.nbody,
                     subtree_com=3, debug=d.dbg_floats, contact_dist=d.ncon, contact_pos=3 * d.ncon, contact_frame=9 * d.ncon)
        unknown = set(out) - set(sizes)
        if unknown:
            raise ValueError(f"unknown rr_outputs field(s): {sorted(unknown)}")
        o = RROutputs()
        for k, w in sizes.items():
            setattr(o, k, _ptr(out.get(k), numel=N * w))
        return o

    def _env(self, env) -> RREnvIOClips:
        d, N = self.dims, self.N
        tp = env["track_pos"]
        clip = env.get("clip")
        if (clip is not None) != (tp.dim() == 3):
            raise ValueError("env io: `clip` goes with a [C, T, 3] track_pos, and only with one")
        e = RREnvIOClips()
        e.track_pos = _ptr(tp)
        e.track_len = tp.shape[-2]
        if clip is not None:
            e.clip = _ptr(clip, torch.int32, N)
            e.num_clips = tp.shape[0]
        e.cur_frame = _ptr(env["cur_frame"], torch.int32, N)
        e.obs = _ptr(env["obs"], numel=N * d.obs_dim)
        e.reward = _ptr(env.get("reward"), numel=N)
# ... 72 lines not shown
        names = ("obs", "raw_action", "log_prob", "reward", "discount", "truncation")
        return RRActorIO(_ptr(obs_in, numel=N * K), _ptr(actor.get("mean"), numel=K), _ptr(actor.get("std"), numel=K), _ptr(actor["w0"]), _ptr(actor["b0"]),
                         hidden(actor["hidden_wt"]), hidden(actor["hidden_b"]), _ptr(actor["head_wt"]), _ptr(actor["head_b"]), _ptr(noise, numel=T * N * A_),
                         _ptr(actions_out, numel=T * N * A_), *(_ptr(traj[k]) if traj is not None else None for k in names), float(actor["min_std"]),
                         len(actor["hidden_wt"]) + 1, int(segment))

    def env_unroll(self, st_in, st_out, actions, n_frames: int, env, cur_frame_in, wrap: dict):
        T = actions.shape[0]
        _check(lib().rr_env_unroll(self.h, C.byref(self._state(st_in)), C.byref(self._state(st_out)),
                                   _ptr(actions, numel=T * self.N * self.dims.nu), T, int(n_frames), C.byref(self._env(env)),
                                   _ptr(cur_frame_in, torch.int32, self.N), C.byref(self._unroll_io(wrap))))

    def env_unroll_policy(self, st_in, st_out, T: int, n_frames: int, env, cur_frame_in, wrap: dict, actor: dict, noise, actions_out, traj: dict,
                          obs_in, segment: int = 0):
        if T % (segment or T):
            raise ValueError("rr_env_unroll_policy: the number of steps must be a multiple of the segment length")
        a = self._actor_io("rr_env_unroll_policy", actor, obs_in, T, noise, actions_out, traj, segment or T)
        _check(lib().rr_env_unroll_policy(self.h, C.byref(self._state(st_in)), C.byref(self._state(st_out)), int(T), int(n_frames),
                                          C.byref(self._env(env)), _ptr(cur_frame_in, torch.int32, self.N), C.byref(self._unroll_io(wrap)), C.byref(a)))

    def eval_supported(self) -> bool:
        return _check(lib().rr_batch_eval_supported(self.h)) == 1

    def env_unroll_eval(self, st_in, st_out, T: int, n_frames: int, env, cur_frame_in, actor: dict, obs_in, obs_ring, noise=None, actions_out=None,
                        eval_metrics=None, qpos_out=None, wrap: Optional[dict] = None):
        d, N = self.dims, self.N
        a = self._actor_io("rr_env_unroll_eval", actor, obs_in, T, noise, actions_out)
        e = RREvalIO(_ptr(eval_metrics, numel=N * 6), _ptr(obs_ring, numel=N * 2 * d.obs_dim), _ptr(qpos_out, numel=(T + 1) * N * d.nq),
                     0 if wrap is not None else 1)
        w = self._unroll_io(wrap) if wrap is not None else None
        _check(lib().rr_env_unroll_eval(self.h, C.byref(self._state(st_in)), C.byref(self._state(st_out)), int(T), int(n_frames), C.byref(self._env(env)),
                                        _ptr(cur_frame_in, torch.int32, N), C.byref(w) if w is not None else None, C.byref(a), C.byref(e)))

    def env_reset(self, st, env, out=None):
        o = self._outputs(out)
        _check(lib().rr_env_reset(self.h, C.byref(self._state(st)), C.byref(self._env(env)), C.byref(o) if o else None))

    def debug_layout(self):
        names, offs, sizes = C.POINTER(C.c_char_p)(), C.POINTER(C.c_int32)(), C.POINTER(C.c_int32)()
        n = _check(lib().rr_debug_layout(self.h, C.byref(names), C.byref(offs), C.byref(sizes)))
        return {names[i].decode(): (offs[i], sizes[i]) for i in range(n)}

    def set_profile(self, buf: Optional[torch.Tensor]):
        _check(lib().rr_batch_set_profile(self.h, _dp(buf)))

    def set_schedule(self, env_map: Optional[torch.Tensor], cost: Optional[torch.Tensor]):
        self._sched = (env_map, cost)
        _check(lib().rr_batch_set_schedule(self.h, _ptr(env_map, torch.int32, self.N), _ptr(cost, torch.int32, self.N)))

    def set_pose(self, track_pose: Optional[torch.Tensor], pose_metrics: Optional[torch.Tensor] = None, quat_reward=(1.0, 2.0), joint_reward=(1.0, 0.5)):
        if track_pose is None:
            _check(lib().rr_batch_set_pose(self.h, None))
            self._pose = None
            return
        p = RRPoseIO(_ptr(track_pose), _ptr(pose_metrics, numel=2 * self.N), *quat_reward, *joint_reward)
        _check(lib().rr_batch_set_pose(self.h, C.byref(p)))
        self._pose = (track_pose, pose_metrics)

    def pose_supported(self) -> Optional[str]:
        if _check(lib().rr_batch_pose_supported(self.h)) == 1:
            return None
        return lib().rr_last_error().decode()

    def env_params_supported(self) -> bool:
        return _check(lib().rr_batch_env_params_supported(self.h)) == 1

    def set_env_params(self, dof_f: Optional[torch.Tensor] = None, act_f: Optional[torch.Tensor] = None, con_f: Optional[torch.Tensor] = None):
        d, N = self.dims, self.N
        for name, t, shape in (("dof_f", dof_f, (N, d.nv, 16)), ("act_f", act_f, (N, d.nu, 8)), ("con_f", con_f, (N, d.ncon, 26))):
            if t is not None and tuple(t.shape) != shape:
                raise ValueError(f"set_env_params: {name} has shape {tuple(t.shape)}, expected {shape}")
        p = RREnvParams(_ptr(dof_f), _ptr(act_f), _ptr(con_f), d.nv, d.nu, d.ncon, N)
        _check(lib().rr_batch_set_env_params(self.h, C.byref(p)))

    def set_ls_repeat_exit(self, enable: bool):
        _check(lib().rr_batch_set_ls_repeat_exit(self.h, int(enable)))

    def set_solver_trim(self, enable: bool):
        _check(lib().rr_batch_set_solver_trim(self.h, int(enable)))

    def set_solver_batch(self, enable: bool):
        _check(lib().rr_batch_set_solver_batch(self.h, int(enable)))

    def set_timing(self, enable: bool):
        _check(lib().rr_batch_set_timing(self.h, int(enable)))

    def kernel_time(self):
        ms, n = C.c_double(), C.c_int64()
        _check(lib().rr_batch_kernel_time(self.h, C.byref(ms), C.byref(n)))
        return ms.value, n.value


def compute_gae(truncation, termination, rewards, values, bootstrap_value, lambda_: float, discount: float):
    T, B = values.shape
    args = [t.contiguous() for t in (truncation, termination, rewards, values, bootstrap_value)]
    for t in args:
        _ptr(t)
    vs = torch.empty_like(args[3])
    adv = torch.empty_like(args[3])
    stream = torch.cuda.current_stream(values.device).cuda_stream
    _check(lib().rr_compute_gae(*[t.data_ptr() for t in args], T, B, float(lambda_), float(discount), vs.data_ptr(),
                                adv.data_ptr(), C.c_void_p(stream)))
    return vs, adv


def wrap_episode_autoreset(first, cur, prev_done, prev_steps, done, steps, truncation, episode_length: float, action_repeat: float):
    n = len(cur)
    N = done.numel()
    for t in list(first) + list(cur) + [prev_done, prev_steps, done, steps, truncation]:
        _ptr(t)
    F = (C.c_void_p * n)(*[t.data_ptr() for t in first])
    Cu = (C.c_void_p * n)(*[t.data_ptr() for t in cur])
    W = (C.c_int32 * n)(*[t.numel() // N for t in cur])
    for f, c in zip(first, cur):
        if f.shape != c.shape:
            raise ValueError("first / current state shapes differ")
    stream = torch.cuda.current_stream(done.device).cuda_stream
    _check(lib().rr_wrap_episode_autoreset(N, n, F, Cu, W, prev_done.data_ptr(), prev_steps.data_ptr(), done.data_ptr(), steps.data_ptr(),
                                           truncation.data_ptr(), float(episode_length), float(action_repeat), C.c_void_p(stream)))


def _mlp_net(weights, biases, in_dim=None):
    n = len(weights)
    for w, b in zip(weights, biases):
        _ptr(w); _ptr(b)
        if w.dim() != 2 or b.numel() != w.shape[0]:
            raise ValueError("weights must be [out, in] with biases [out]")
    W = (C.c_void_p * n)(*[w.data_ptr() for w in weights])
    B = (C.c_void_p * n)(*[b.data_ptr() for b in biases])
    S = (C.c_int32 * (n + 1))(in_dim or weights[0].shape[1], *[w.shape[0] for w in weights])
    return RRMlpNet(C.cast(W, C.POINTER(C.c_void_p)), C.cast(B, C.POINTER(C.c_void_p)), C.cast(S, C.POINTER(C.c_int32)), n), (W, B, S)


def mlp_forward(obs, mean=None, std=None, policy=None, value=None, want_pre=False, rows=None):
    M, K = obs.shape
    _ptr(obs)
    if rows is not None:
        M = rows.numel()
        _ptr(rows, torch.int64)
    dev = obs.device
    pn = vn = None
    keep = []
    pol_out = val_out = pol_pre = val_pre = None
    if policy is not None:
        pn, k = _mlp_net(*policy, in_dim=K); keep.append((k, policy))
        pol_out = torch.empty(M, policy[0][-1].shape[0], device=dev)
        if want_pre:
            pol_pre = torch.empty(len(policy[0]) - 1, M, policy[0][0].shape[0], device=dev)
    if value is not None:
        vn, k = _mlp_net(*value, in_dim=K); keep.append((k, value))
        val_out = torch.empty(M, device=dev)
        if want_pre:
            val_pre = torch.empty(len(value[0]) - 1, M, 256, device=dev)
    stream = torch.cuda.current_stream(dev).cuda_stream
    _check(lib().rr_mlp_forward(obs.data_ptr(), _dp(rows), M, K, _ptr(mean, numel=K), _ptr(std, numel=K), C.byref(pn) if pn is not None else None,
                                C.byref(vn) if vn is not None else None, _dp(pol_out), _dp(val_out), _dp(pol_pre), _dp(val_pre), C.c_void_p(stream)))
    return pol_out, val_out, pol_pre, val_pre


def ppo_loss(policy_logits, values, data, idx, noise, T: int, *, entropy_cost, discounting, reward_scaling, gae_lambda, clipping_epsilon,
             normalize_advantage=True, min_std=0.001, out=None):
    M, P2 = policy_logits.shape
    B = M // (T + 1)
    A = P2 // 2
    dev = policy_logits.device
    for t in (policy_logits, values, noise, data["raw_action"], data["log_prob"], data["reward"], data["discount"], data["truncation"]):
# ... 175 lines not shown
```

include/rodent_rr.h:

```cpp
#ifndef RODENT_RR_H
#define RODENT_RR_H
#include <stddef.h>
#include <stdint.h>

#ifdef __cplusplus
extern "C" {
#endif

typedef struct rr_model rr_model;
typedef struct rr_batch rr_batch;

enum rr_status { RR_OK = 0, RR_EINVAL = -1, RR_EIO = -2, RR_EHIP = -3, RR_EUNSUPPORTED = -4 };

typedef struct rr_dims {
  int32_t nq, nv, nu, na, nbody, njnt, ngeom, nM, ncon, nlimit, nefc, obs_dim;
  int32_t iterations, ls_iterations;
  int32_t lds_bytes;
  int32_t dbg_floats;
  float timestep;
  int32_t solver;
  int32_t fixed_instance;
} rr_dims;

typedef struct rr_state {
// ... 116 lines not shown
} rr_mlp_net;
int rr_mlp_forward(const float* obs, const int64_t* obs_rows, int32_t M, int32_t K, const float* mean, const float* std, const rr_mlp_net* policy,
                   const rr_mlp_net* value, float* policy_out, float* value_out, float* policy_pre, float* value_pre, void* stream);


typedef struct rr_ppo_cfg {
  float entropy_cost, discounting, reward_scaling, gae_lambda, clipping_epsilon, min_std;
  int32_t normalize_advantage;
} rr_ppo_cfg;
size_t rr_ppo_loss_workspace_bytes(int32_t T, int32_t B);
int rr_ppo_loss(const float* policy_logits, const float* values, const float* raw_action, const float* log_prob, const float* reward,
                const float* discount, const float* truncation, const int64_t* idx, const float* noise, int32_t T, int32_t B, int32_t A,
                const rr_ppo_cfg* cfg, float* grad_logits, float* grad_values, float* metrics, void* workspace, size_t workspace_bytes,
                void* stream);

size_t rr_policy_act_workspace_bytes(int32_t M);
int rr_policy_act(const float* obs, const int64_t* obs_rows, int32_t M, int32_t K, const float* mean, const float* std,
                  const rr_mlp_net* policy, const float* noise, float min_std, float* action, float* raw_action, float* log_prob,
                  float* logits, void* workspace, size_t workspace_bytes, void* stream);

int rr_policy_sample(const float* logits, const float* noise, int32_t N, int32_t A, float min_std, float* action, float* raw_action,
                     float* log_prob, void* stream);

size_t rr_policy_backward_workspace_bytes(int32_t M, int32_t nhidden);
int rr_policy_backward(const float* grad_logits, const float* head_weight, const float* const* hidden_weights, int32_t nhidden, int32_t M,
                       int32_t P, float* pre_act, int32_t pre_act_rows, float* delta, float* const* bias_grads, void* workspace,
                       size_t workspace_bytes, void* stream);

size_t rr_mlp_silu_backward_workspace_bytes(int32_t M, int32_t H);
int rr_mlp_silu_backward(const float* g, const float* z, int32_t M, int32_t H, float* delta, float* h, float* bias_grad,
                         void* workspace, size_t workspace_bytes, void* stream);

size_t rr_mlp_value_backward_workspace_bytes(int32_t M, int32_t nhidden);
int rr_mlp_value_backward(const float* grad_value, const float* head_weight, const float* const* hidden_weights_t, int32_t nhidden,
                          int32_t M, float* pre_act, float* delta, float* const* bias_grads, void* workspace, size_t workspace_bytes,
                          void* stream);

size_t rr_mlp_policy_backward_workspace_bytes(int32_t n, int32_t nhidden);
int rr_mlp_policy_backward(const float* grad_logits, const float* head_weight_t, const float* const* hidden_weights_t, int32_t nhidden,
                           int32_t n, int32_t M, int32_t P, float* pre_act, float* delta, float* const* bias_grads, void* workspace,
                           size_t workspace_bytes, void* stream);

size_t rr_mlp_weight_grad_workspace_bytes(int32_t M, int32_t O, int32_t I);
int rr_mlp_weight_grad(const float* delta, const float* act, const int64_t* act_rows, const float* mean, const float* std,
                       const float* delta_colsum, int32_t M, int32_t O, int32_t I, float* grad, void* workspace, size_t workspace_bytes,
                       void* stream);

typedef struct rr_dw_item {
  const float* delta; const float* act; const int64_t* act_rows; const float* mean; const float* std; const float* delta_colsum;
  int32_t M, O, I;
  float* grad;
} rr_dw_item;
size_t rr_mlp_weight_grad_batch_workspace_bytes(const rr_dw_item* items, int32_t n);
int rr_mlp_weight_grad_batch(const rr_dw_item* items, int32_t n, void* workspace, size_t workspace_bytes, void* stream);

size_t rr_obs_moments_workspace_bytes(int64_t nseq, int32_t T, int32_t K);
int rr_obs_moments(const float* obs, int64_t nseq, int32_t Tp1, int32_t T, int32_t K, const float* mean, double* sums, void* workspace,
                   size_t workspace_bytes, void* stream);

int rr_wrap_episode_autoreset(int32_t num_envs, int32_t narr, const float* const* first, float* const* cur, const int32_t* widths,
                              const float* prev_done, const float* prev_steps, float* done, float* steps, float* truncation,
                              float episode_length, float action_repeat, void* stream);

int rr_batch_set_schedule(rr_batch* b, const int32_t* env_map, uint32_t* cost_cycles);

typedef struct rr_env_params {
  const float* dof_f;
  const float* act_f;
  const float* con_f;
  int32_t dof_rows, act_rows, con_rows;
  int32_t num_envs;
} rr_env_params;
int rr_batch_set_env_params(rr_batch* b, const rr_env_params* p);
int rr_batch_env_params_supported(const rr_batch* b);

int rr_debug_layout(const rr_batch* b, const char*** names, const int32_t** offsets, const int32_t** sizes);

int rr_batch_set_ls_repeat_exit(rr_batch* b, int32_t enable);

int rr_batch_set_solver_trim(rr_batch* b, int32_t enable);

int rr_batch_set_solver_batch(rr_batch* b, int32_t enable);

int rr_batch_set_timing(rr_batch* b, int32_t enable);
int rr_batch_kernel_time(rr_batch* b, double* total_ms, int64_t* launches);

int rr_batch_set_profile(rr_batch* b, uint64_t* dev_cycles);

int rr_kernarg_layout(int32_t* io_offset, int32_t* io_size, int32_t* total_size);

const char* rr_last_error(void);

#ifdef __cplusplus
}
#endif
#endif
```

Measured before the change: 1.926 million.

## Pair factorisation row ops via host-side dependency scheduler into fewer rows

```diff
diff --git a/__graft_entry__.py b/__graft_entry__.py
--- a/__graft_entry__.py
+++ b/__graft_entry__.py
@@ -12,7 +12,7 @@
 def build() -> None:
     csrc = os.path.join(PKG, "csrc")
     so = os.path.join(csrc, "librodent_hip.so")
-    srcs = [os.path.join(csrc, f) for f in ("rr_api.hip", "rr_kernel.h", "rr_step_body.inc", "rr_mlp.h", "rr_ppo.h", "rr_tanh_normal.h")] + [os.path.join(ROOT, "include", "rodent_rr.h")]
+    srcs = [os.path.join(csrc, f) for f in ("rr_api.hip", "rr_kernel.h", "rr_pairsched.h", "rr_step_body.inc", "rr_mlp.h", "rr_ppo.h", "rr_tanh_normal.h")] + [os.path.join(ROOT, "include", "rodent_rr.h")]
     if not os.path.exists(so) or any(os.path.getmtime(s) > os.path.getmtime(so) for s in srcs):
         cmd = ["hipcc", "--offload-arch=gfx950", "-O2", "-std=c++17", "-shared", "-fPIC", "-fno-slp-vectorize", "-Xclang", "-target-feature",
                "-Xclang", "-load-store-opt", "-o", so, os.path.join(csrc, "rr_api.hip")]
diff --git a/brax-rodent-run_amd/csrc/rr_api.hip b/brax-rodent-run_amd/csrc/rr_api.hip
--- a/brax-rodent-run_amd/csrc/rr_api.hip
+++ b/brax-rodent-run_amd/csrc/rr_api.hip
@@ -2,6 +2,7 @@
 #include "rr_kernel.h"
 #include "rr_mlp.h"
 #include "rr_ppo.h"
+#include "rr_pairsched.h"
 
 #include <atomic>
 #include <climits>
@@ -43,6 +44,8 @@
   bool pair_ok = false;
   RRDims kd_rep;
   bool dyn = false;
+  mutable std::map<std::string, rr_pairsched::Program> paired;
+  mutable std::mutex paired_mu;
   mutable std::atomic<int> live_batches{0};
 
   const Entry* find(const char* n) const { auto it = e.find(n); return it == e.end() ? nullptr : &it->second; }
@@ -106,6 +109,24 @@
   return Instance{family((RRDims*)nullptr)};
 }
 
+static const rr_pairsched::Program* paired_program(const rr_model* m, const char* name) {
+  std::lock_guard<std::mutex> lk(m->paired_mu);
+  auto it = m->paired.find(name);
+  if (it != m->paired.end()) return &it->second;
+  const bool rep = !strncmp(name, "h_", 2);
+  const Entry *e = m->find(name), *er = m->find((std::string(name) + "_rows").c_str()), *hd = m->find("h_dims");
+  if (!e || !er || !er->count || (rep && (!hd || hd->count < 8))) return nullptr;
+  const int32_t* h = rep ? (const int32_t*)hd->data : nullptr;
+  const int nrows = ((const int32_t*)er->data)[0];
+  if (nrows < 0 || e->count < (size_t)nrows * RR_LANES * 4) return nullptr;
+  const rr_dims& d = m->dims;
+  const RRLayout L = rep ? rr_layout(h[0], h[1], h[2], h[3], h[5], h[6], false) : rr_layout(d.nq, d.nv, d.nu, d.nbody, d.nM, m->dyn ? m->NCS * RR_LANES : d.ncon, false);
+  rr_pairsched::Slots S;
+  S.nM = (uint32_t)(rep ? h[5] : d.nM); S.matrix_slot = (uint32_t)L.o_qLD / 2; S.alias_slot = (uint32_t)L.o_xpos / 2;
+  return &(m->paired[name] = rr_pairsched::derive((const uint32_t*)e->data, nrows, S.nM, S));
+}
+static int paired_ints(const rr_pairsched::Program& P) { return (P.nrows + rr_pairsched::RING) * RR_LANES * 5; }
+
 static void set_layout(RRDims& k, const RRLayout& L) {
   k.o_qpos = L.o_qpos; k.o_qvel = L.o_qvel; k.o_act = L.o_act; k.o_ctrl = L.o_ctrl; k.o_xpos = L.o_xpos; k.o_xquat = L.o_xquat;
   k.o_cinert = L.o_cinert; k.o_cdof = L.o_cdof; k.o_cvel = L.o_cvel; k.o_qLD = L.o_qLD; k.o_vec = L.o_vec; k.o_x = L.o_x;
@@ -128,7 +149,11 @@
   const RRLayout L = rr_layout(d.nq, d.nv, d.nu, d.nbody, d.nM, con_slots, m->solver == 2);
   set_layout(k, L);
   k.solver = m->solver;
-  k.nfac = m->iscalar(m->solver == 2 ? "k_factor3p_rows" : "k_factor3_rows");
+  k.nfac = k.nfac_blob = m->iscalar(m->solver == 2 ? "k_factor3p_rows" : "k_factor3_rows");
+  k.fac_blob_off = 0;
+#if RR_FACTOR_PAIRED
+  if (const rr_pairsched::Program* P = paired_program(m, m->solver == 2 ? "k_factor3p" : "k_factor3")) { k.nfac = P->nrows; k.fac_blob_off = paired_ints(*P); }
+#endif
   k.nalias = m->solver == 2 ? 0 : m->iscalar("k_nalias");
   m->dbg_names.clear(); m->dbg_off.clear(); m->dbg_size.clear(); m->dbg_cnames.clear();
   m->stage_ok = stage_fits(d.nbody, d.nv, con_slots, k.nalias);
@@ -179,6 +204,11 @@
   k.nv_scale = m->dims.nv;
   k.lds_bytes_rep = L.lds_floats * 4;
   k.fac_stride = (int)m->find("h_k_factor3")->count; k.inv_stride = (int)m->find("h_k_linv")->count;
+  k.nfac_blob = k.nfac; k.fac_blob_off = 0;
+#if RR_FACTOR_PAIRED
+  if (const rr_pairsched::Program* P = paired_program(m, "h_k_factor3")) { k.nfac = P->nrows; k.fac_stride = paired_ints(*P); }
+  else return;
+#endif
   if (!solve_jobs_fit(m, "h_", 2 * RR_LANES, k)) return;
   if (k.nM > RR_LANES * 18 || k.nroot != 1) return;
   if (!stage_fits(k.nbody, k.nv, k.ncon, k.nalias) || 2 * k.lds_bytes_rep + 128 > 64 * 1024) return;
@@ -297,6 +327,16 @@
   if (dtype) *dtype = e->dtype;
   return RR_OK;
 }
+extern "C" int rr_model_factor_paired(const rr_model* m, const char* name, int32_t* rows, const uint32_t** words, size_t* count, int32_t* paired) {
+  if (!m || !name) return fail(RR_EINVAL, "rr_model_factor_paired: null argument");
+  const rr_pairsched::Program* P = paired_program(m, name);
+  if (!P) return fail(RR_EINVAL, std::string("rr_model_factor_paired: the model has no row program '") + name + "'");
+  if (rows) *rows = P->nrows;
+  if (words) *words = P->words.data();
+  if (count) *count = P->words.size();
+  if (paired) *paired = P->paired ? 1 : 0;
+  return RR_OK;
+}
 extern "C" int rr_kernarg_layout(int32_t* io_offset, int32_t* io_size, int32_t* total_size) {
   if (io_offset) *io_offset = (int32_t)offsetof(RRKArgs, io);
   if (io_size) *io_size = (int32_t)sizeof(RRIO);
@@ -346,26 +386,58 @@
   return dev_alloc(b, std::max<size_t>(e->count, 1) * 4, dst, e->data, e->count * 4);
 }
 
+static int levels_to_lds(const Entry* e, uint32_t* tc, uint32_t cb, uint32_t ab, uint32_t nM) {
+  const uint32_t* src = (const uint32_t*)e->data;
+  for (size_t i = 0; i + 3 < e->count; i += 4) {
+    uint32_t f[6] = {src[i] & 0xFFFFu, src[i] >> 16, src[i + 1] & 0xFFFFu, src[i + 1] >> 16, src[i + 2] & 0xFFFFu, src[i + 2] >> 16};
+    for (uint32_t& v : f) {
+      v = v < nM + 4u ? v * 8u + cb : (v - (nM + 4u)) * 8u + ab;
+      if (v > 0xFFFFu) return fail(RR_EUNSUPPORTED, "level schedule does not fit the 16-bit LDS address fields");
+    }
+    const uint32_t q = src[i + 3];
+    if (q > 255u) return fail(RR_EIO, "level schedule: pivot offset out of range (stale blob)");
+    tc[i] = f[0] | (f[1] << 16); tc[i + 1] = f[2] | (f[3] << 16); tc[i + 2] = f[4] | (f[5] << 16);
+    tc[i + 3] = q * 8u;
+  }
+  return RR_OK;
+}
 static int upload_levels(rr_batch* b, const char* name, rr_gi* dst, uint32_t base, uint32_t alias_base, uint32_t nM, int copies = 1, uint32_t rep_bytes = 0) {
   const Entry* e = b->m->find(name);
   std::vector<uint32_t> t((size_t)copies * e->count);
+  for (int c = 0; c < copies; ++c)
+    if (int rc = levels_to_lds(e, t.data() + (size_t)c * e->count, base + (uint32_t)c * rep_bytes, alias_base + (uint32_t)c * rep_bytes, nM)) return rc;
+  return dev_alloc(b, t.size() * 4, dst, t.data(), t.size() * 4);
+}
+static int upload_factor(rr_batch* b, const char* name, rr_gi* dst, uint32_t base, uint32_t alias_base, uint32_t nM, int copies, uint32_t rep_bytes, bool with_blob) {
+#if RR_FACTOR_PAIRED
+  const rr_pairsched::Program* P = paired_program(b->m, name);
+  if (!P) return fail(RR_EIO, "factorisation schedule: no row program to pair");
+  const Entry* e = b->m->find(name);
+  const size_t per = (size_t)paired_ints(*P), nlane = (size_t)(P->nrows + rr_pairsched::RING) * RR_LANES;
+  std::vector<uint32_t> t(per * copies + (with_blob ? e->count : 0));
   for (int c = 0; c < copies; ++c) {
-    const uint32_t* src = (const uint32_t*)e->data;
-    uint32_t* tc = t.data() + (size_t)c * e->count;
     const uint32_t cb = base + (uint32_t)c * rep_bytes, ab = alias_base + (uint32_t)c * rep_bytes;
-    for (size_t i = 0; i + 3 < e->count; i += 4) {
-      uint32_t f[6] = {src[i] & 0xFFFFu, src[i] >> 16, src[i + 1] & 0xFFFFu, src[i + 1] >> 16, src[i + 2] & 0xFFFFu, src[i + 2] >> 16};
+    for (size_t ln = 0; ln < nlane; ++ln) {
+      const uint32_t* w = P->words.data() + ln * rr_pairsched::WORDS;
+      uint32_t* row = t.data() + c * per + ln / RR_LANES * (RR_LANES * 5);
+      uint32_t f[8] = {w[0] & 0xFFFFu, w[0] >> 16, w[1] & 0xFFFFu, w[1] >> 16, w[2] & 0xFFFFu, w[2] >> 16, w[3] & 0xFFFFu, w[3] >> 16};
       for (uint32_t& v : f) {
-        v = v < nM + 4u ? v * 8u + cb : (v - (nM + 4u)) * 8u + ab;
+        v = v >= rr_pairsched::ZRUN ? (nM + 4u + (v - rr_pairsched::ZRUN)) * 8u + cb : (v < nM + 4u ? v * 8u + cb : (v - (nM + 4u)) * 8u + ab);
         if (v > 0xFFFFu) return fail(RR_EUNSUPPORTED, "level schedule does not fit the 16-bit LDS address fields");
       }
-      const uint32_t q = src[i + 3];
-      if (q > 255u) return fail(RR_EIO, "level schedule: pivot offset out of range (stale blob)");
-      tc[i] = f[0] | (f[1] << 16); tc[i + 1] = f[2] | (f[3] << 16); tc[i + 2] = f[4] | (f[5] << 16);
-      tc[i + 3] = q * 8u;
+      if (w[4] > 255u || w[5] > 255u) return fail(RR_EIO, "level schedule: pivot offset out of range (stale blob)");
+      uint32_t* x = row + (ln % RR_LANES) * 4;
+      for (int k = 0; k < 4; ++k) x[k] = f[2 * k] | (f[2 * k + 1] << 16);
+      row[RR_LANES * 4 + ln % RR_LANES] = (w[4] * 8u) | ((w[5] * 8u) << 16);
     }
   }
+  if (with_blob)
+    if (int rc = levels_to_lds(e, t.data() + per * copies, base, alias_base, nM)) return rc;
   return dev_alloc(b, t.size() * 4, dst, t.data(), t.size() * 4);
+#else
+  (void)with_blob;
+  return upload_levels(b, name, dst, base, alias_base, nM, copies, rep_bytes);
+#endif
 }
 
 static int lds_bytes(const rr_model* m, Variant v) { return v == V_PAIR ? 2 * m->kd_rep.lds_bytes_rep + 128 : m->dims.lds_bytes; }
@@ -387,13 +459,13 @@
   UP_REPLICA_TABLES(b->T, "")
   UP(b->T, "", act_i) UP(b->T, "", act_m_i) UP(b->T, "", act_m_f)
   const uint32_t qb = (uint32_t)m->kd.o_qLD * 4u, ab = (uint32_t)m->kd.o_xpos * 4u, nM = (uint32_t)m->dims.nM;
-  if ((rc = upload_levels(b, m->solver == 2 ? "k_factor3p" : "k_factor3", &b->T.factor3, qb, ab, nM)) || (rc = upload_levels(b, "k_linv", &b->T.linv, qb, ab, nM))) return rc;
+  if ((rc = upload_factor(b, m->solver == 2 ? "k_factor3p" : "k_factor3", &b->T.factor3, qb, ab, nM, 1, 0, true)) || (rc = upload_levels(b, "k_linv", &b->T.linv, qb, ab, nM))) return rc;
   memset(&b->T_rep, 0, sizeof(b->T_rep));
   if (m->pair_ok) {
     UP_REPLICA_TABLES(b->T_rep, "h_")
     const uint32_t base = (uint32_t)m->kd_rep.o_qLD * 4u, rb = (uint32_t)m->kd_rep.lds_bytes_rep;
     const uint32_t abase = (uint32_t)m->kd_rep.o_xpos * 4u, hnM = (uint32_t)m->kd_rep.nM;
-    if ((rc = upload_levels(b, "h_k_factor3", &b->T_rep.factor3, base, abase, hnM, 2, rb)) || (rc = upload_levels(b, "h_k_linv", &b->T_rep.linv, base, abase, hnM, 2, rb))) return rc;
+    if ((rc = upload_factor(b, "h_k_factor3", &b->T_rep.factor3, base, abase, hnM, 2, rb, false)) || (rc = upload_levels(b, "h_k_linv", &b->T_rep.linv, base, abase, hnM, 2, rb))) return rc;
     b->T_rep.anc4 = b->T_rep.M_ij_k;
   }
 #undef UP_REPLICA_TABLES
@@ -1292,6 +1364,12 @@
   return RR_OK;
 }
 
+extern "C" int rr_batch_set_factor_paired(rr_batch* b, int32_t enable) {
+  if (!b) return fail(RR_EINVAL, "rr_batch_set_factor_paired: null batch");
+  b->dbg_flags = enable ? (b->dbg_flags & ~RR_DBG_FACTOR_UNPAIRED) : (b->dbg_flags | RR_DBG_FACTOR_UNPAIRED);
+  return RR_OK;
+}
+
 extern "C" int rr_batch_set_timing(rr_batch* b, int32_t enable) {
   if (!b) return fail(RR_EINVAL, "rr_batch_set_timing: null batch");
   HIPCHK(hipSetDevice(b->device));
diff --git a/brax-rodent-run_amd/csrc/rr_kernel.h b/brax-rodent-run_amd/csrc/rr_kernel.h
--- a/brax-rodent-run_amd/csrc/rr_kernel.h
+++ b/brax-rodent-run_amd/csrc/rr_kernel.h
@@ -36,6 +36,12 @@
 #endif
 #ifndef RR_LS_STAGE_ONCE
 #define RR_LS_STAGE_ONCE 1
+#endif
+#ifndef RR_FACTOR_PAIRED
+#define RR_FACTOR_PAIRED 1
+#endif
+#ifndef RR_PAIR_RING_SHIFT
+#define RR_PAIR_RING_SHIFT 4
 #endif
 #define RR_MINVAL 1e-15f
 #define RR_MINIMP 0.0001f
@@ -50,6 +56,7 @@
   int o_H, o_Mp, o_anc, solver;
   int nv_scale, fac_stride, inv_stride, lds_bytes_rep;
   int nalias;
+  int nfac_blob, fac_blob_off;
   int g_xpos, g_xquat, g_xmat, g_com, g_cinert, g_crb, g_cdof, g_cvel, g_cfrc, g_qM, g_qLD, g_dinv, g_bias, g_passive,
       g_actuator, g_smooth, g_qacc_smooth, g_con_dist, g_con_pos, g_con_frame, g_con_D, g_con_aref, g_lim, g_qacc,
       g_qfrc_constraint, g_misc, g_ls_iters, g_solver_end, g_kaok, dbg_floats;
@@ -189,6 +196,7 @@
 #define RR_DBG_LS_RUN_REPEATS 1
 #define RR_DBG_SOLVER_UNTRIMMED 2
 #define RR_DBG_SOLVER_UNBATCHED 4
+#define RR_DBG_FACTOR_UNPAIRED 8
 struct v3 { float x, y, z; };
 __device__ __forceinline__ v3 mk3(float x, float y, float z) { v3 r; r.x = x; r.y = y; r.z = z; return r; }
 __device__ __forceinline__ v3 ld3(const float* p) { return mk3(p[0], p[1], p[2]); }
@@ -983,12 +991,79 @@
     }
   }
 
-  __device__ __forceinline__ void factor() {
+  struct PairAdr { int a8[2], p8[2], b8[2], d8[4]; };
+  template <bool SHIFT>
+  static __device__ __forceinline__ PairAdr pair_adr(const rr_v4i& e, int q, int delta) {
+    const int sh = SHIFT ? delta : 0;
+    PairAdr r;
+    r.a8[0] = (e.x & 0xFFFF) + sh; r.b8[0] = (int)((unsigned)e.x >> 16) + sh;
+    r.a8[1] = (e.y & 0xFFFF) + sh; r.b8[1] = (int)((unsigned)e.y >> 16) + sh;
+    r.p8[0] = r.a8[0] - (q & 0xFFFF) + 8; r.p8[1] = r.a8[1] - (int)((unsigned)q >> 16) + 8;
+    r.d8[0] = (e.z & 0xFFFF) + sh; r.d8[1] = (int)((unsigned)e.z >> 16) + sh; r.d8[2] = (e.w & 0xFFFF) + sh; r.d8[3] = (int)((unsigned)e.w >> 16) + sh;
+    return r;
+  }
+  static constexpr int PAIR_ROW_INTS = RR_LANES * 5;
+  template <bool SHIFT = false, int RING = RR_RING>
+  __device__ __forceinline__ void run_pairs(rr_gi table, int nrows, int delta = 0) {
+    typedef const rr_v4i __attribute__((address_space(1)))* rr_gv4;
+    typedef const int __attribute__((address_space(1)))* rr_g1;
+    typedef const char __attribute__((address_space(1)))* rr_gc;
+    const rr_gc tab = (rr_gc)table;
+    const unsigned lane16 = 16u * (unsigned)lane, lane4 = RR_LANES * 16u + 4u * (unsigned)lane;
+    constexpr int ROWB = PAIR_ROW_INTS * 4;
+    rr_v4i ring[RING];
+    int ringq[RING];
+#pragma unroll
+    for (int u = 0; u < RING; ++u) { ring[u] = *(rr_gv4)(tab + u * ROWB + lane16); ringq[u] = *(rr_g1)(tab + u * ROWB + lane4); }
+    PairAdr cur = pair_adr<SHIFT>(ring[0], ringq[0], delta);
+    for (int r0 = 0; r0 < nrows; r0 += RING) {
+      const rr_gc nxt_rows = tab + (size_t)(r0 + RING) * ROWB;
+#pragma unroll
+      for (int u = 0; u < RING; ++u) {
+        if (u && r0 + u >= nrows) break;
+        const rr_f2 va1 = lds_ld2(cur.a8[0]), vp1 = lds_ld2(cur.p8[0]), va2 = lds_ld2(cur.a8[1]), vp2 = lds_ld2(cur.p8[1]);
+        rr_f2 vb1[4], vb2[4], vo[4];
+#pragma unroll
+        for (int j = 0; j < 4; ++j) vb1[j] = lds_ld2(cur.b8[0] + 8 * j);
+#pragma unroll
+        for (int j = 0; j < 4; ++j) vb2[j] = lds_ld2(cur.b8[1] + 8 * j);
+#pragma unroll
+        for (int j = 0; j < 4; ++j) vo[j] = lds_ld2(cur.d8[j]);
+        ring[u] = *(rr_gv4)(nxt_rows + u * ROWB + lane16);
+        ringq[u] = *(rr_g1)(nxt_rows + u * ROWB + lane4);
+        const PairAdr nxt = pair_adr<SHIFT>(ring[(u + 1) % RING], ringq[(u + 1) % RING], delta);
+        rr_f2 r1 = {__builtin_amdgcn_rcpf(vp1.x), __builtin_amdgcn_rcpf(vp1.y)}, r2 = {__builtin_amdgcn_rcpf(vp2.x), __builtin_amdgcn_rcpf(vp2.y)};
+        r1 = r1 * (2.0f - vp1 * r1); r2 = r2 * (2.0f - vp2 * r2);
+        rr_f2 t1 = va1, t2 = va2;
+        t1 *= r1; t2 *= r2;
+#pragma unroll
+        for (int j = 0; j < 4; ++j) {
+          const rr_f2 first = vo[j] - vb1[j] * t1;
+          lds_st2(cur.d8[j], first - vb2[j] * t2);
+        }
+        cur = nxt;
+      }
+    }
+  }
+  template <bool SHIFT, bool DBG>
+  __device__ __forceinline__ void run_factor(int flags, int delta = 0) {
+#if RR_FACTOR_PAIRED
+    if constexpr (DBG) {
+      if (flags & RR_DBG_FACTOR_UNPAIRED) { run_levels<true, SHIFT>(TL.factor3 + D.fac_blob_off, D.nfac_blob, delta); return; }
+    }
+    run_pairs<SHIFT, SHIFT ? RR_PAIR_RING_SHIFT : RR_RING>(PAIR ? TL.factor3 + rep * D.fac_stride : TL.factor3, D.nfac, delta);
+#else
+    run_levels<true, SHIFT>(PAIR ? TL.factor3 + rep * D.fac_stride : TL.factor3, D.nfac, delta);
+#endif
+  }
+
+  template <bool DBG = false>
+  __device__ __forceinline__ void factor(int flags = 0) {
     int ment[NME];
     load_ment(ment);
     const RRTables T = tables();
     const DT D = phase_dims();
-    if (lane < 8) s_qLD[2 * D.nM + lane] = (lane >> 1) == 1 ? 1.0f : ((lane >> 1) == 3 ? -1.0f : 0.0f);
+    if (lane < 16) s_qLD[2 * D.nM + lane] = (lane >> 1) == 1 ? 1.0f : ((lane >> 1) == 3 ? -1.0f : 0.0f);
     for (int c = lane; c < 2 * D.nalias; c += RR_LANES) s_buf[c] = 0.0f;
 #pragma unroll
     for (int s = 0; s < NVS; ++s) {
@@ -996,7 +1071,7 @@
       if (d < D.nv) s_qLD[2 * (opaque(dofc1[s]) & 0xFFFF) + 1] += D.dt * row_at(T.dof_f, 16, d)[1];
     }
     sync();
-    run_levels<true>(PAIR ? TL.factor3 + rep * D.fac_stride : TL.factor3, D.nfac);
+    run_factor<false, DBG>(flags);
     sync();
 #pragma unroll
     for (int s = 0; s < NVS; ++s) {
@@ -1675,13 +1750,14 @@
       }
     }
   }
+  template <bool DBG = false>
   __device__ __forceinline__ void newton_factor() {
     const int delta = (int)((D.o_H - D.o_qLD) * sizeof(float));
     int ment[NME];
     load_ment(ment);
-    if (lane < 8) s_H[2 * D.nM + lane] = (lane >> 1) == 1 ? 1.0f : 0.0f;
-    sync();
-    run_levels<true, true>(TL.factor3, D.nfac, delta);
+    if (lane < 16) s_H[2 * D.nM + lane] = (lane >> 1) == 1 ? 1.0f : 0.0f;
+    sync();
+    run_factor<true, DBG>(dbg_flags, delta);
     sync();
 #pragma unroll
     for (int s = 0; s < NVS; ++s) {
@@ -1707,13 +1783,14 @@
 #pragma unroll
     for (int s = 0; s < NVS; ++s) grad[s] = Ma[s] - qfrc_smooth[s] - qfrc_con[s];
   }
+  template <bool DBG = false>
   __device__ __forceinline__ void solve_gradient() {
 #pragma unroll
     for (int s = 0; s < NVS; ++s) Mgrad[s] = grad[s];
     for (int rep = 0; rep < RR_REP_SOLVE; ++rep) { float t_[NVS]; for (int s = 0; s < NVS; ++s) t_[s] = grad[s]; ldl_solve(t_); }
     if (NEWTON) {
       newton_hessian();
-      newton_factor();
+      newton_factor<DBG>();
       ldl_solve_on(Mgrad, s_H, dinvH);
     } else {
       ldl_solve(Mgrad);
@@ -2023,7 +2100,7 @@
 #pragma unroll
     for (int s = 0; s < NVS; ++s) pm[s] = 0.0f;
     while (true) {
-      if (untrimmed) { solve_gradient(); direction(niter, pm, gg); }
+      if (untrimmed) { solve_gradient<DBG>(); direction(niter, pm, gg); }
       const float improvement = (prev_cost - cost) * scale;
       float g2 = 0.0f;
 #pragma unroll
@@ -2038,7 +2115,7 @@
       }
       if constexpr (PROF) { if (niter) stamp<PROF>(12); }
       if (!untrimmed) {
-        solve_gradient();
+        solve_gradient<DBG>();
         if constexpr (PROF) { if (niter) stamp<PROF>(11); }
         direction(niter, pm, gg);
       }
diff --git a/brax-rodent-run_amd/csrc/rr_pairsched.h b/brax-rodent-run_amd/csrc/rr_pairsched.h
--- /dev/null
+++ b/brax-rodent-run_amd/csrc/rr_pairsched.h
@@ -0,0 +1,317 @@
+#ifndef RR_PAIRSCHED_H
+#define RR_PAIRSCHED_H
+#include <algorithm>
+#include <array>
+#include <cstdint>
+#include <map>
+#include <set>
+#include <utility>
+#include <vector>
+
+namespace rr_pairsched {
+
+constexpr int LANES = 64, WORDS = 6, RING = 8;
+constexpr uint32_t ZRUN = 0xFFF0u;
+
+struct Program {
+  int nrows = 0;
+  bool paired = false;
+  std::vector<uint32_t> words;
+};
+struct Slots {
+  uint32_t nM = 0, matrix_slot = 0, alias_slot = 0;
+  uint32_t slot(uint32_t e) const { return e >= ZRUN ? matrix_slot + nM + 4 + (e - ZRUN) : (e < nM + 4 ? matrix_slot + e : alias_slot + e - (nM + 4)); }
+};
+
+namespace detail {
+struct InOp { uint32_t a, b0, q, d[4]; int row; };
+struct Versions {
+  std::vector<std::array<int, 6>> rv;
+  std::vector<std::array<int, 4>> ord;
+  std::vector<int> nw;
+  bool ok = true;
+};
+struct Joined { int h[2]; };
+
+inline std::vector<InOp> parse(const uint32_t* w, int nrows, uint32_t nM) {
+  const uint32_t TRASH = nM + 2;
+  std::vector<InOp> ops;
+  for (int r = 0; r < nrows; ++r)
+    for (int l = 0; l < LANES; ++l) {
+      const uint32_t* e = w + ((size_t)r * LANES + l) * 4;
+      InOp o{e[0] & 0xFFFFu, e[0] >> 16, e[3], {e[1] & 0xFFFFu, e[1] >> 16, e[2] & 0xFFFFu, e[2] >> 16}, r};
+      if (o.d[0] == TRASH && o.d[1] == TRASH && o.d[2] == TRASH && o.d[3] == TRASH) continue;
+      ops.push_back(o);
+    }
+  return ops;
+}
+inline uint32_t source(const InOp& o, int k) { return k == 0 ? o.a : (k == 1 ? o.a + 1 - o.q : o.b0 + (uint32_t)(k - 2)); }
+inline bool source_matters(const InOp& o, int k, uint32_t nM) { return k < 2 || o.d[k - 2] != nM + 2; }
+
+inline Versions versions(const std::vector<InOp>& ops, uint32_t nM, size_t ncell) {
+  const uint32_t TRASH = nM + 2;
+  Versions V;
+  V.rv.resize(ops.size()); V.ord.resize(ops.size()); V.nw.assign(ncell, 0);
+  for (size_t t0 = 0; t0 < ops.size();) {
+    size_t t1 = t0;
+    while (t1 < ops.size() && ops[t1].row == ops[t0].row) ++t1;
+    for (size_t t = t0; t < t1; ++t) {
+      for (int k = 0; k < 6; ++k) V.rv[t][k] = source_matters(ops[t], k, nM) ? V.nw[source(ops[t], k)] : -1;
+      for (int j = 0; j < 4; ++j) V.ord[t][j] = ops[t].d[j] == TRASH ? 0 : V.nw[ops[t].d[j]] + 1;
+    }
+    for (size_t t = t0; t < t1; ++t)
+      for (int j = 0; j < 4; ++j)
+        if (ops[t].d[j] != TRASH) {
+          if (V.nw[ops[t].d[j]] + 1 != V.ord[t][j]) V.ok = false;
+          ++V.nw[ops[t].d[j]];
+        }
+    t0 = t1;
+  }
+  return V;
+}
+
+inline void emit_half(uint32_t* w, int h, const InOp* o, uint32_t nM) {
+  w[h] = o ? (o->a | (o->b0 << 16)) : (nM | (ZRUN << 16));
+  w[4 + h] = o ? o->q : 0u;
+}
+inline void emit_empty(uint32_t* w, uint32_t nM) {
+  const uint32_t T = nM + 2;
+  emit_half(w, 0, nullptr, nM); emit_half(w, 1, nullptr, nM);
+  w[2] = w[3] = T | (T << 16);
+}
+inline void emit(uint32_t* w, const InOp* o1, const InOp* o2, uint32_t nM) {
+  emit_half(w, 0, o1, nM); emit_half(w, 1, o2, nM);
+  w[2] = o1->d[0] | (o1->d[1] << 16); w[3] = o1->d[2] | (o1->d[3] << 16);
+}
+
+inline std::array<int, LANES> assign_lanes(const std::vector<int>& row, const std::vector<Joined>& J, const std::vector<InOp>& ops, const Slots& S) {
+  std::map<uint32_t, std::vector<int>> cls;
+  for (int t : row) cls[S.slot(ops[J[t].h[0]].d[0]) & 15u].push_back(t);
+  std::vector<std::pair<uint32_t, const std::vector<int>*>> order;
+  for (auto& kv : cls) order.push_back({kv.first, &kv.second});
+  std::stable_sort(order.begin(), order.end(), [](const auto& x, const auto& y) { return x.second->size() > y.second->size(); });
+  std::vector<int> Q[4], over;
+  for (auto& kv : order) {
+    int qs[4] = {0, 1, 2, 3};
+    std::stable_sort(qs, qs + 4, [&](int x, int y) { return Q[x].size() < Q[y].size(); });
+    for (size_t i = 0; i < kv.second->size(); ++i) {
+      if (i < 4 && Q[qs[i]].size() < 16) Q[qs[i]].push_back((*kv.second)[i]);
+      else over.push_back((*kv.second)[i]);
+    }
+  }
+  for (int t : over) {
+    int q = 0;
+    for (int x = 1; x < 4; ++x) if (Q[x].size() < Q[q].size()) q = x;
+    Q[q].push_back(t);
+  }
+  std::array<int, LANES> lanes;
+  lanes.fill(-1);
+  for (int q = 0; q < 4; ++q)
+    for (size_t i = 0; i < Q[q].size() && i < 16; ++i) lanes[16 * q + (int)i] = Q[q][i];
+  return lanes;
+}
+
+struct Graph {
+  int n = 0;
+  std::vector<std::vector<int>> raw, war, raw_succ, war_succ;
+  std::vector<int> tail;
+  bool ok = true;
+};
+
+inline std::vector<std::vector<int>> list_schedule(const Graph& g, const std::vector<int>& group, int ngroup, double w) {
+  const int n = g.n;
+  std::vector<int> nraw(n), row_of(n, -1), remaining(ngroup, 0), ready;
+  for (int t = 0; t < n; ++t) { nraw[t] = (int)g.raw[t].size(); ++remaining[group[t]]; if (!nraw[t]) ready.push_back(t); }
+  std::vector<std::vector<int>> rows;
+  int done = 0;
+  while (done < n) {
+    std::vector<std::pair<double, int>> keyed;
+    for (int t : ready) keyed.push_back({-(g.tail[t] + w * (remaining[group[t]] - 1)), t});
+    std::sort(keyed.begin(), keyed.end());
+    std::vector<int> cand, row;
+    for (auto& kt : keyed) cand.push_back(kt.second);
+    std::vector<char> used(ngroup, 0);
+    bool progress = true;
+    while (progress && (int)row.size() < LANES) {
+      progress = false;
+      std::vector<int> rest;
+      for (int t : cand) {
+        bool can = (int)row.size() < LANES && !used[group[t]];
+        for (size_t i = 0; can && i < g.war[t].size(); ++i) can = row_of[g.war[t][i]] >= 0;
+        if (!can) { rest.push_back(t); continue; }
+        row_of[t] = (int)rows.size(); row.push_back(t); used[group[t]] = 1; --remaining[group[t]];
+        progress = true;
+      }
+      cand.swap(rest);
+    }
+    if (row.empty()) return {};
+    ready.swap(cand);
+    for (int t : row)
+      for (int s : g.raw_succ[t]) if (--nraw[s] == 0) ready.push_back(s);
+    done += (int)row.size();
+    rows.push_back(row);
+  }
+  return rows;
+}
+
+inline bool check(const Program& P, const std::vector<InOp>& ops, const Versions& V, uint32_t nM, size_t ncell) {
+  const uint32_t ZERO = nM, TRASH = nM + 2;
+  if (P.words.size() != (size_t)(P.nrows + RING) * LANES * WORDS) return false;
+  std::map<std::array<uint32_t, 7>, std::vector<int>> by_word;
+  for (int t = (int)ops.size() - 1; t >= 0; --t) by_word[{ops[t].a, ops[t].b0, ops[t].q, ops[t].d[0], ops[t].d[1], ops[t].d[2], ops[t].d[3]}].push_back(t);
+  std::vector<int> ver(ncell, 0), stamp(ncell, -1);
+  size_t seen = 0;
+  for (int r = 0; r < P.nrows + RING; ++r) {
+    std::vector<std::pair<uint32_t, int>> writes;
+    for (int l = 0; l < LANES; ++l) {
+      const uint32_t* w = P.words.data() + ((size_t)r * LANES + l) * WORDS;
+      const uint32_t d[4] = {w[2] & 0xFFFFu, w[2] >> 16, w[3] & 0xFFFFu, w[3] >> 16};
+      const bool empty = d[0] == TRASH && d[1] == TRASH && d[2] == TRASH && d[3] == TRASH;
+      int k = 0;
+      for (int h = 0; h < 2; ++h) {
+        const uint32_t a = w[h] & 0xFFFFu, b0 = w[h] >> 16, q = w[4 + h];
+        if (a == ZERO && b0 == ZRUN && q == 0) continue;
+        if (empty || r >= P.nrows || (h == 1 && k == 0)) return false;
+        auto it = by_word.find({a, b0, q, d[0], d[1], d[2], d[3]});
+        if (it == by_word.end() || it->second.empty()) return false;
+        const int t = it->second.back();
+        it->second.pop_back(); ++seen;
+        for (int s = 0; s < 6; ++s) if (V.rv[t][s] >= 0 && ver[source(ops[t], s)] != V.rv[t][s]) return false;
+        for (int j = 0; j < 4; ++j) if (d[j] != TRASH && ver[d[j]] + k + 1 != V.ord[t][j]) return false;
+        ++k;
+      }
+      if (k) for (int j = 0; j < 4; ++j) if (d[j] != TRASH) writes.push_back({d[j], k});
+    }
+    for (auto& cw : writes) {
+      if (stamp[cw.first] == r) return false;
+      stamp[cw.first] = r; ver[cw.first] += cw.second;
+    }
+  }
+  return seen == ops.size();
+}
+
+inline Program singles(const std::vector<InOp>& ops, const uint32_t* w, int nrows, uint32_t nM) {
+  Program P;
+  P.nrows = nrows; P.paired = false;
+  P.words.resize((size_t)(nrows + RING) * LANES * WORDS);
+  for (size_t i = 0; i < P.words.size(); i += WORDS) emit_empty(&P.words[i], nM);
+  const uint32_t TRASH = nM + 2;
+  size_t t = 0;
+  for (int r = 0; r < nrows; ++r)
+    for (int l = 0; l < LANES; ++l) {
+      const uint32_t* e = w + ((size_t)r * LANES + l) * 4;
+      if ((e[1] & 0xFFFFu) == TRASH && (e[1] >> 16) == TRASH && (e[2] & 0xFFFFu) == TRASH && (e[2] >> 16) == TRASH) continue;
+      emit(&P.words[((size_t)r * LANES + l) * WORDS], &ops[t], nullptr, nM); ++t;
+    }
+  return P;
+}
+}
+
+inline Program derive(const uint32_t* w, int nrows, uint32_t nM, const Slots& S) {
+  using namespace detail;
+  const uint32_t TRASH = nM + 2;
+  const std::vector<InOp> ops = parse(w, nrows, nM);
+  size_t ncell = nM + 8;
+  for (const InOp& o : ops) {
+    if (o.q > o.a + 1) return singles(ops, w, nrows, nM);
+    ncell = std::max<size_t>(ncell, std::max({o.a, o.b0 + 3, o.d[0], o.d[1], o.d[2], o.d[3]}) + 1);
+  }
+  if (ncell > ZRUN) return singles(ops, w, nrows, nM);
+  const Versions V = versions(ops, nM, ncell);
+  const Program fallback = singles(ops, w, nrows, nM);
+  if (!V.ok) return fallback;
+  const int n_in = (int)ops.size();
+
+  std::set<std::pair<uint32_t, int>> needed;
+  for (int t = 0; t < n_in; ++t)
+    for (int k = 0; k < 6; ++k) if (V.rv[t][k] > 0) needed.insert({source(ops[t], k), V.rv[t][k]});
+  std::map<std::array<uint32_t, 4>, std::vector<int>> tuples;
+  for (int t = 0; t < n_in; ++t) tuples[{ops[t].d[0], ops[t].d[1], ops[t].d[2], ops[t].d[3]}].push_back(t);
+  std::vector<Joined> J;
+  std::vector<int> group;
+  int ngroup = 0;
+  for (auto& kv : tuples) {
+    const std::vector<int>& ts = kv.second;
+    for (size_t i = 0; i < ts.size();) {
+      bool join = i + 1 < ts.size();
+      for (int j = 0; join && j < 4; ++j)
+        if (kv.first[j] != TRASH) join = V.ord[ts[i + 1]][j] == V.ord[ts[i]][j] + 1 && !needed.count({kv.first[j], V.ord[ts[i]][j]});
+      J.push_back(join ? Joined{{ts[i], ts[i + 1]}} : Joined{{ts[i], -1}});
+      group.push_back(ngroup);
+      i += join ? 2 : 1;
+    }
+    ++ngroup;
+  }
+  const int n = (int)J.size();
+
+  std::vector<std::vector<int>> writer(ncell);
+  for (size_t c = 0; c < ncell; ++c) writer[c].assign(V.nw[c], -1);
+  for (int t = 0; t < n; ++t)
+    for (int h = 0; h < 2; ++h) if (J[t].h[h] >= 0)
+      for (int j = 0; j < 4; ++j) { const InOp& o = ops[J[t].h[h]]; if (o.d[j] != TRASH) writer[o.d[j]][V.ord[J[t].h[h]][j] - 1] = t; }
+  Graph g;
+  g.n = n; g.raw.resize(n); g.war.resize(n); g.raw_succ.resize(n); g.war_succ.resize(n);
+  for (int t = 0; t < n; ++t) {
+    for (int h = 0; h < 2; ++h) if (J[t].h[h] >= 0) {
+      const int i = J[t].h[h];
+      for (int k = 0; k < 6; ++k) {
+        const int v = V.rv[i][k];
+        if (v < 0) continue;
+        const uint32_t c = source(ops[i], k);
+        if (v > 0 && writer[c][v - 1] != t) g.raw[t].push_back(writer[c][v - 1]);
+        if (v < V.nw[c] && writer[c][v] != t) g.war[writer[c][v]].push_back(t);
+      }
+    }
+    const int i = J[t].h[0];
+    for (int j = 0; j < 4; ++j) if (ops[i].d[j] != TRASH && V.ord[i][j] > 1) g.raw[t].push_back(writer[ops[i].d[j]][V.ord[i][j] - 2]);
+  }
+  for (int t = 0; t < n; ++t) {
+    for (auto* e : {&g.raw[t], &g.war[t]}) { std::sort(e->begin(), e->end()); e->erase(std::unique(e->begin(), e->end()), e->end()); }
+    for (int d : g.raw[t]) g.raw_succ[d].push_back(t);
+    for (int d : g.war[t]) g.war_succ[d].push_back(t);
+  }
+  {
+    std::vector<int> indeg(n), order, stack;
+    for (int t = 0; t < n; ++t) { indeg[t] = (int)(g.raw[t].size() + g.war[t].size()); if (!indeg[t]) stack.push_back(t); }
+    while (!stack.empty()) {
+      const int t = stack.back(); stack.pop_back(); order.push_back(t);
+      for (auto* e : {&g.raw_succ[t], &g.war_succ[t]}) for (int s : *e) if (--indeg[s] == 0) stack.push_back(s);
+    }
+    if ((int)order.size() != n) return fallback;
+    g.tail.assign(n, 0);
+    for (int i = n - 1; i >= 0; --i) {
+      const int t = order[i];
+      for (int s : g.raw_succ[t]) g.tail[t] = std::max(g.tail[t], g.tail[s] + 1);
+      for (int s : g.war_succ[t]) g.tail[t] = std::max(g.tail[t], g.tail[s]);
+    }
+  }
+  std::vector<std::vector<int>> best;
+  for (double wgt : {0.75, 1.0, 2.0, 0.5, 0.25}) {
+    std::vector<std::vector<int>> rows = list_schedule(g, group, ngroup, wgt);
+    if (!rows.empty() && (best.empty() || rows.size() < best.size())) best.swap(rows);
+  }
+  if (best.empty() || (int)best.size() > nrows) return fallback;
+
+  Program P;
+  P.nrows = (int)best.size(); P.paired = true;
+  P.words.resize((size_t)(P.nrows + RING) * LANES * WORDS);
+  for (size_t i = 0; i < P.words.size(); i += WORDS) emit_empty(&P.words[i], nM);
+  for (int r = 0; r < P.nrows; ++r) {
+    const std::array<int, LANES> lanes = assign_lanes(best[r], J, ops, S);
+    for (int l = 0; l < LANES; ++l)
+      if (lanes[l] >= 0) emit(&P.words[((size_t)r * LANES + l) * WORDS], &ops[J[lanes[l]].h[0]], J[lanes[l]].h[1] >= 0 ? &ops[J[lanes[l]].h[1]] : nullptr, nM);
+  }
+  return check(P, ops, V, nM, ncell) ? P : fallback;
+}
+
+inline bool verify(const Program& P, const uint32_t* w, int nrows, uint32_t nM) {
+  using namespace detail;
+  const std::vector<InOp> ops = parse(w, nrows, nM);
+  size_t ncell = nM + 8;
+  for (const InOp& o : ops) ncell = std::max<size_t>(ncell, std::max({o.a, o.b0 + 3, o.d[0], o.d[1], o.d[2], o.d[3]}) + 1);
+  const Versions V = versions(ops, nM, ncell);
+  return V.ok && check(P, ops, V, nM, ncell);
+}
+
+}
+#endif
diff --git a/brax-rodent-run_amd/csrc/rr_step_body.inc b/brax-rodent-run_amd/csrc/rr_step_body.inc
--- a/brax-rodent-run_amd/csrc/rr_step_body.inc
+++ b/brax-rodent-run_amd/csrc/rr_step_body.inc
@@ -198,7 +198,8 @@
     if ((w.lag_mode & 8) && w.lag_prio == 0) __builtin_amdgcn_s_setprio(2);
     else __builtin_amdgcn_s_setprio(3);
 #endif
-    w.factor();
+    w.template factor<DBG>(DBG ? io.dbg_flags : 0);
+    w.template stamp<PROF>(22);
     if (dg) for (int e = lane; e < D.nM; e += RR_LANES) dg[D.g_qLD + e] = w.s_qLD[2 * e];
     w.invert();
     w.env_prio();
diff --git a/brax-rodent-run_amd/rodent_amd/hip.py b/brax-rodent-run_amd/rodent_amd/hip.py
--- a/brax-rodent-run_amd/rodent_amd/hip.py
+++ b/brax-rodent-run_amd/rodent_amd/hip.py
@@ -75,7 +75,7 @@
         [("normalize_advantage", C.c_int32)]
 
 
-EXPORTS = ["rr_model_load", "rr_model_dims", "rr_model_set_solver", "rr_model_set_solver_type", "rr_model_destroy", "rr_model_table", "rr_kernarg_layout", "rr_batch_create",
+EXPORTS = ["rr_model_load", "rr_model_dims", "rr_model_set_solver", "rr_model_set_solver_type", "rr_model_destroy", "rr_model_table", "rr_model_factor_paired", "rr_batch_set_factor_paired", "rr_kernarg_layout", "rr_batch_create",
            "rr_batch_destroy", "rr_pipeline_init", "rr_pipeline_step", "rr_env_step", "rr_env_reset", "rr_pipeline_step_to", "rr_env_step_to", "rr_batch_contact_overflow", "rr_batch_bad_states", "rr_batch_unroll_supported", "rr_env_unroll", "rr_env_unroll_policy", "rr_batch_eval_supported", "rr_env_unroll_eval", "rr_batch_pose_supported", "rr_batch_set_pose",
            "rr_compute_gae", "rr_mlp_forward", "rr_ppo_loss_workspace_bytes", "rr_ppo_loss", "rr_policy_act_workspace_bytes", "rr_policy_act", "rr_policy_sample", "rr_policy_backward_workspace_bytes", "rr_policy_backward", "rr_mlp_silu_backward_workspace_bytes", "rr_mlp_silu_backward", "rr_mlp_value_backward_workspace_bytes", "rr_mlp_policy_backward", "rr_mlp_policy_backward_workspace_bytes", "rr_mlp_value_backward", "rr_mlp_weight_grad_workspace_bytes", "rr_mlp_weight_grad", "rr_mlp_weight_grad_batch_workspace_bytes", "rr_mlp_weight_grad_batch", "rr_obs_moments_workspace_bytes", "rr_obs_moments", "rr_wrap_episode_autoreset", "rr_debug_layout", "rr_batch_set_schedule", "rr_batch_set_env_params", "rr_batch_env_params_supported", "rr_batch_set_profile", "rr_batch_set_ls_repeat_exit", "rr_batch_set_solver_trim", "rr_batch_set_solver_batch", "rr_batch_set_timing", "rr_batch_kernel_time", "rr_last_error"]
 
@@ -96,6 +96,7 @@
         L.rr_model_destroy.argtypes = [C.c_void_p]
         L.rr_model_destroy.restype = None
         L.rr_model_table.argtypes = [C.c_void_p, C.c_char_p, C.POINTER(C.c_void_p), C.POINTER(C.c_size_t), C.POINTER(C.c_int32)]
+        L.rr_model_factor_paired.argtypes = [C.c_void_p, C.c_char_p, C.POINTER(C.c_int32), C.POINTER(C.c_void_p), C.POINTER(C.c_size_t), C.POINTER(C.c_int32)]
         L.rr_kernarg_layout.argtypes = [C.POINTER(C.c_int32)] * 3
         L.rr_batch_create.argtypes = [C.c_void_p, C.c_int32, C.c_int32, C.c_void_p, C.POINTER(C.c_void_p)]
         L.rr_batch_destroy.argtypes = [C.c_void_p]
@@ -166,6 +167,7 @@
         L.rr_batch_set_ls_repeat_exit.argtypes = [C.c_void_p, C.c_int32]
         L.rr_batch_set_solver_trim.argtypes = [C.c_void_p, C.c_int32]
         L.rr_batch_set_solver_batch.argtypes = [C.c_void_p, C.c_int32]
+        L.rr_batch_set_factor_paired.argtypes = [C.c_void_p, C.c_int32]
         L.rr_batch_set_timing.argtypes = [C.c_void_p, C.c_int32]
         L.rr_batch_kernel_time.argtypes = [C.c_void_p, C.POINTER(C.c_double), C.POINTER(C.c_int64)]
         _lib = L
@@ -218,6 +220,13 @@
         if iterations is not None:
             d = self.dims
             _check(lib().rr_model_set_solver(self.h, iterations, ls_iterations if ls_iterations is not None else d.ls_iterations))
+
+    def factor_paired(self, name: str = "k_factor3"):
+        import numpy as np
+        rows, ptr, cnt, pr = C.c_int32(), C.c_void_p(), C.c_size_t(), C.c_int32()
+        _check(lib().rr_model_factor_paired(self.h, name.encode(), C.byref(rows), C.byref(ptr), C.byref(cnt), C.byref(pr)))
+        w = np.ctypeslib.as_array(C.cast(ptr, C.POINTER(C.c_uint32)), shape=(cnt.value,)).copy()
+        return rows.value, w.reshape(-1, 64, 6), bool(pr.value)
 
     def table(self, name: str):
         import numpy as np
@@ -456,6 +465,9 @@
     def set_solver_batch(self, enable: bool):
         _check(lib().rr_batch_set_solver_batch(self.h, int(enable)))
 
+    def set_factor_paired(self, enable: bool):
+        _check(lib().rr_batch_set_factor_paired(self.h, int(enable)))
+
     def set_timing(self, enable: bool):
         _check(lib().rr_batch_set_timing(self.h, int(enable)))
 
diff --git a/include/rodent_rr.h b/include/rodent_rr.h
--- a/include/rodent_rr.h
+++ b/include/rodent_rr.h
@@ -222,6 +222,10 @@
 
 int rr_batch_set_solver_batch(rr_batch* b, int32_t enable);
 
+int rr_batch_set_factor_paired(rr_batch* b, int32_t enable);
+
+int rr_model_factor_paired(const rr_model* m, const char* name, int32_t* rows, const uint32_t** words, size_t* count, int32_t* paired);
+
 int rr_batch_set_timing(rr_batch* b, int32_t enable);
 int rr_batch_kernel_time(rr_batch* b, double* total_ms, int64_t* launches);
 
```

Measured after the change: 1.930 million (median of 4 runs). About the same (+0.2%).
